# peterropac/Aegolius

Measured on AMD Instinct MI355X. Metric: Mpoints/sec SDF eval, 1024^3 grid, 10-prim smooth-union tree, higher is better.
Workload: dtype f32

## Files before the change

aegolius_amd/_engine.py:

```python
import atexit
import contextlib
import ctypes
import importlib.util
import os
import sys
import threading

import numpy as np

_HERE = os.path.dirname(os.path.abspath(__file__))
LIB_PATH = os.path.join(_HERE, "libsdfk.so")

MODE_AUTO, MODE_INTERPRET, MODE_SPECIALIZED, MODE_NOCULL = 0, 1, 2, 3
(FLAVOUR_PLAIN_ARRAY, FLAVOUR_PLAIN_GRID, FLAVOUR_TILE_ARRAY, FLAVOUR_TILE_GRID, FLAVOUR_TILE_MASK, FLAVOUR_ROWS_ARRAY,
 FLAVOUR_ROWS_GRID, FLAVOUR_ROWS_MASK, FLAVOUR_ROWS2D_ARRAY, FLAVOUR_ROWS2D_GRID, FLAVOUR_RAYS, FLAVOUR_OCCUPANCY) = range(12)
FLAVOUR_FLAGS = 0x100
FLAVOUR_XY = 0x200

_c = ctypes
_vp, _i64, _int, _sz = _c.c_void_p, _c.c_int64, _c.c_int, _c.c_size_t
_fp = _c.POINTER(_c.c_float)

SIGNATURES = {
    "sdfk_abi_version": (_int, []),
    "sdfk_device_count": (_int, []),
    "sdfk_last_error": (_c.c_char_p, []),
    "sdfk_program_create": (_vp, [_vp, _sz, _vp, _sz, _vp, _sz, _int]),
    "sdfk_program_destroy": (None, [_vp]),
    "sdfk_program_set_params": (_int, [_vp, _vp, _sz]),
    "sdfk_program_set_cull": (_int, [_vp, _vp, _sz, _vp]),
    "sdfk_program_source": (_c.c_char_p, [_vp]),
    "sdfk_program_compile_check": (_int, [_vp, _c.POINTER(_sz)]),
    "sdfk_program_chain_members": (_int, [_vp]),
    "sdfk_program_compile_flavour": (_int, [_vp, _int, _c.POINTER(_sz), _c.POINTER(_c.c_double)]),
    "sdfk_debug_compile_external": (_int, [_vp, _int, _c.POINTER(_sz)]),
    "sdfk_debug_jit_stats": (None, [_c.POINTER(_i64), _c.POINTER(_c.c_double)]),
    "sdfk_jit_drain": (None, []),
    "sdfk_jit_cancel": (None, []),
    "sdfk_debug_set_rtc_defs": (None, [_c.c_char_p]),
    "sdfk_eval_device": (_int, [_vp, _vp, _i64, _i64, _vp, _vp, _int]),
    "sdfk_eval_device_rows": (_int, [_vp, _vp, _i64, _i64, _i64, _vp, _vp, _int]),
    "sdfk_eval_device_rows2d": (_int, [_vp, _vp, _i64, _i64, _i64, _vp, _vp, _int]),
    "sdfk_eval_device_rows2d_xy": (_int, [_vp, _vp, _i64, _i64, _i64, _vp, _vp, _int]),
    "sdfk_debug_cells_stats": (None, [_int, _c.POINTER(_c.c_longlong)]),
    "sdfk_debug_rays_stats": (None, [_int, _c.POINTER(_c.c_longlong)]),
    "sdfk_eval_device_rows3d": (_int, [_vp, _vp, _i64, _i64, _i64, _i64, _i64, _vp, _vp, _int]),
    "sdfk_debug_row_masks": (_int, [_vp, _vp, _i64, _i64, _i64, _vp, _c.POINTER(_i64), _c.POINTER(_int), _vp]),
    "sdfk_eval_grid_sharded": (_int, [_vp, _vp, _i64, _vp, _i64, _vp, _i64, _int, _vp, _vp, _int]),
    "sdfk_eval_grid_sharded_device": (_int, [_vp, _vp, _i64, _vp, _i64, _vp, _i64, _int, _vp, _int, _vp, _int]),
    "sdfk_eval_device_aux": (_int, [_vp, _vp, _i64, _i64, _vp, _int, _i64, _vp, _vp, _int]),
    "sdfk_eval_grid_aux": (_int, [_vp, _vp, _i64, _vp, _i64, _vp, _i64, _i64, _i64, _vp, _int, _i64, _vp, _vp, _int]),
    "sdfk_field_min": (_int, [_vp, _i64, _c.POINTER(_c.c_float), _vp]),
    "sdfk_grid_box_average": (_int, [_vp, _i64, _i64, _i64, _int, _int, _int, _int, _vp, _vp]),
    "sdfk_grid_edge_detect": (_int, [_vp, _i64, _i64, _i64, _vp, _vp]),
    "sdfk_debug_box_variant": (_int, [_i64, _i64, _i64, _int, _int, _int, _c.POINTER(_int)]),
    "sdfk_grid_signed": (_int, [_vp, _i64, _i64, _i64, _c.c_float, _int, _vp, _vp]),
    "sdfk_grid_boundary_mask": (_int, [_vp, _i64, _c.c_float, _vp, _vp]),
    "sdfk_grid_signed_slab": (_int, [_vp, _i64, _i64, _vp, _i64, _i64, _i64, _int, _vp, _vp]),
    "sdfk_eval_host": (_int, [_vp, _vp, _int, _i64, _i64, _vp, _int, _int]),
    "sdfk_eval_host_resident": (_int, [_vp, _vp, _int, _i64, _i64, _vp, _int, _int]),
    "sdfk_field_select_scratch": (_sz, [_i64]),
    "sdfk_field_select": (_int, [_vp, _i64, _c.c_float, _vp, _i64, _c.POINTER(_i64), _vp, _vp]),
    "sdfk_field_select_finish": (_int, [_i64, _i64, _vp, _i64, _vp, _vp]),
    "sdfk_field_gradient": (_int, [_vp, _i64, _i64, _i64, _int, _int, _vp, _i64, _vp]),
    "sdfk_field_crossings_2d": (_int, [_vp, _vp, _i64, _i64, _i64, _c.c_double, _c.c_double, _c.c_double, _vp, _vp]),
    "sdfk_lcwg_eval": (_int, [_int, _vp, _vp, _i64, _i64, _i64, _c.c_double, _c.c_double, _int, _c.c_double, _vp, _vp, _i64,
                              _vp]),
    "sdfk_lcwg_old_eval": (_int, [_int, _vp, _i64, _vp, _i64, _c.c_double, _c.c_double, _vp, _i64, _vp]),
    "sdfk_eval_select_scratch": (_sz, [_i64, _i64]),
    "sdfk_eval_device_select": (_int, [_vp, _vp, _i64, _i64, _i64, _int, _c.c_float, _vp, _i64, _c.POINTER(_i64), _vp, _vp, _int]),
    "sdfk_eval_grid_select": (_int, [_vp, _vp, _i64, _vp, _i64, _vp, _i64, _i64, _i64, _c.c_float, _vp, _i64, _c.POINTER(_i64),
                                     _vp, _vp, _int]),
    "sdfk_eval_select_finish": (_int, [_vp, _i64, _i64, _int, _i64, _vp, _i64, _vp, _vp]),
    "sdfk_vec_eval_device": (_int, [_vp, _int, _vp, _i64, _i64, _vp, _int, _i64, _int, _vp, _i64, _vp]),
    "sdfk_vec_set_interpret": (None, [_int]),
    "sdfk_vec_source": (_c.c_char_p, [_vp, _int, _int, _int]),
    "sdfk_vec_compile_check": (_int, [_vp, _int, _int, _int, _c.POINTER(_sz)]),
    "sdfk_vec_eval_host": (_int, [_vp, _int, _vp, _int, _i64, _vp, _i64, _vp, _i64, _vp, _i64, _vp, _int, _int, _vp, _int]),
    "sdfk_eval_grid": (_int, [_vp, _vp, _i64, _vp, _i64, _vp, _i64, _i64, _i64, _vp, _vp, _int]),
    "sdfk_eval_grid_host": (_int, [_vp, _vp, _i64, _vp, _i64, _vp, _i64, _i64, _i64, _vp, _int, _int]),
    "sdfk_set_default_mode": (None, [_int]),
    "sdfk_debug_brick_masks": (_int, [_vp, _vp, _i64, _i64, _vp, _vp]),
    "sdfk_linspace_f32": (_int, [_c.c_double, _c.c_double, _i64, _vp]),
    "sdfk_point_tree_build": (_i64, [_vp, _i64, _int, _vp, _i64, _vp, _vp, _vp]),
    "sdfk_grid_fill": (_int, [_vp, _i64, _vp, _i64, _vp, _i64, _vp, _i64, _i64, _i64, _vp]),
    "sdfk_set_device": (_int, [_int]),
    "sdfk_malloc": (_vp, [_sz]),
    "sdfk_free": (_int, [_vp]),
    "sdfk_memcpy_h2d": (_int, [_vp, _vp, _sz]),
    "sdfk_memcpy_d2h": (_int, [_vp, _vp, _sz]),
    "sdfk_memcpy_d2d": (_int, [_vp, _vp, _sz]),
    "sdfk_sync": (_int, [_vp]),
    "sdfk_event_create": (_vp, []),
    "sdfk_event_destroy": (_int, [_vp]),
    "sdfk_event_record": (_int, [_vp, _vp]),
    "sdfk_event_elapsed_ms": (_int, [_vp, _vp, _fp]),
    "sdfk_stream_probe": (_int, [_vp, _i64, _i64, _vp, _vp]),
    "sdfk_dual_has_rule": (_int, [_int]),
    "sdfk_program_jvp_check": (_int, [_vp, _c.POINTER(_int)]),
    "sdfk_eval_jvp_device": (_int, [_vp, _vp, _i64, _i64, _vp, _int, _int, _vp, _vp, _i64, _vp]),
    "sdfk_value_jvp_device": (_int, [_int, _vp, _vp, _vp, _i64, _vp, _vp, _vp]),
    "sdfk_program_vjp_check": (_int, [_vp, _c.POINTER(_int), _c.POINTER(_i64)]),
    "sdfk_vjp_limits": (_int, [_c.POINTER(_int), _c.POINTER(_int)]),
    "sdfk_eval_vjp_device": (_int, [_vp, _vp, _i64, _i64, _vp, _int, _int, _vp, _vp, _vp, _vp]),
    "sdfk_points_bin": (_int, [_vp, _i64, _i64, _vp, _i64, _i64, _i64, _vp, _vp]),
    "sdfk_points_extent": (_int, [_vp, _i64, _i64, _i64, _vp, _vp]),
    "sdfk_points_fill": (_int, [_vp, _i64, _i64, _i64, _int, _i64, _i64, _i64, _vp]),
    "sdfk_points_widen": (_int, [_vp, _i64, _int, _vp, _vp]),
    "sdfk_field_isosurface_scratch": (_sz, [_i64, _i64, _i64]),
    "sdfk_field_isosurface": (_int, [_vp, _vp, _i64, _vp, _i64, _vp, _i64, _c.c_float, _c.POINTER(_i64), _c.POINTER(_i64), _vp,
                                     _vp]),
    "sdfk_field_isosurface_finish": (_int, [_vp, _i64, _i64, _i64, _c.c_float, _i64, _i64, _vp, _i64, _vp, _i64, _int, _vp,
                                            _vp]),
    "sdfk_field_contour2d_scratch": (_sz, [_i64, _i64]),
    "sdfk_field_contour2d": (_int, [_vp, _vp, _i64, _vp, _i64, _c.c_float, _c.POINTER(_i64), _c.POINTER(_i64), _vp, _vp]),
    "sdfk_field_contour2d_finish": (_int, [_vp, _i64, _i64, _c.c_float, _i64, _i64, _vp, _i64, _vp, _i64, _int, _vp, _vp]),
    "sdfk_eval_grid_isosurface_scratch": (_sz, [_i64, _i64, _i64]),
    "sdfk_eval_grid_isosurface": (_int, [_vp, _vp, _i64, _vp, _i64, _vp, _i64, _c.c_float, _c.POINTER(_i64), _c.POINTER(_i64),
                                         _vp, _vp, _int]),
    "sdfk_eval_grid_isosurface_finish": (_int, [_vp, _vp, _i64, _vp, _i64, _vp, _i64, _c.c_float, _i64, _i64, _vp, _i64, _vp,
                                                _i64, _int, _vp, _vp, _int]),
    "sdfk_eval_grid_contour2d_scratch": (_sz, [_i64, _i64]),
    "sdfk_eval_grid_contour2d": (_int, [_vp, _vp, _i64, _vp, _i64, _c.c_float, _c.POINTER(_i64), _c.POINTER(_i64), _vp, _vp,
                                        _int]),
    "sdfk_eval_grid_contour2d_finish": (_int, [_vp, _vp, _i64, _vp, _i64, _c.c_float, _i64, _i64, _vp, _i64, _vp, _i64, _int,
                                               _vp, _vp, _int]),
    "sdfk_program_rays_check": (_int, [_vp, _c.POINTER(_int)]),
    "sdfk_trace_rays_device": (_int, [_vp, _vp, _i64, _vp, _i64, _i64, _c.c_float, _c.c_float, _c.c_float, _c.c_float,
                                      _c.c_float, _int, _vp, _vp, _vp, _vp, _i64, _vp, _int]),
    "sdfk_trace_camera_device": (_int, [_vp, _vp, _int, _int, _int, _c.c_float, _c.c_float, _c.c_float, _c.c_float,
                                        _c.c_float, _int, _vp, _vp, _vp, _vp, _i64, _vp, _int]),
    "sdfk_eval_grid_occupancy_scratch": (_sz, [_i64, _i64, _i64, _i64]),
    "sdfk_eval_grid_occupancy": (_int, [_vp, _vp, _i64, _vp, _i64, _vp, _i64, _vp, _vp, _vp, _vp, _vp, _vp, _int, _c.c_float,
                                        _c.c_float, _vp, _vp, _i64, _c.POINTER(_i64), _c.POINTER(_i64), _fp, _vp, _int]),
    "sdfk_field_row_sums": (_int, [_vp, _i64, _i64, _vp, _vp, _vp]),
    "sdfk_field_redistance_scratch": (_sz, [_i64, _i64, _i64]),
    "sdfk_field_redistance": (_int, [_vp, _vp, _i64, _vp, _i64, _vp, _i64, _c.c_float, _c.c_float, _int, _vp, _vp,
                                     _c.POINTER(_i64), _fp, _vp]),
}


class SdfkError(RuntimeError):
    pass


_lib = None
_lock = threading.Lock()


def _share_torch_hip_runtime():
    if "torch" in sys.modules:
        return
    try:
        spec = importlib.util.find_spec("torch")
    except (ImportError, ValueError):
        spec = None
    if spec is None or not spec.submodule_search_locations:
        return
    libdir = os.path.join(list(spec.submodule_search_locations)[0], "lib")
    for name in ("libamdhip64.so", "libhiprtc.so"):
        path = os.path.join(libdir, name)
        if os.path.exists(path):
            try:
                ctypes.CDLL(path, mode=ctypes.RTLD_GLOBAL)
            except OSError:
# ... 617 lines not shown
```

aegolius_amd/csrc/sdfk.hip:

```cpp
#include <hip/hip_runtime.h>
#include <hip/hiprtc.h>

#include <chrono>
#include <algorithm>
#include <atomic>
#include <cmath>
#include <condition_variable>
#include <cstdio>
#include <cstdlib>
#include <cstring>
#include <deque>
#include <functional>
#include <map>
#include <memory>
#include <mutex>
#include <thread>
#include <string>
#include <vector>
#include <dirent.h>
#include <dlfcn.h>
#include <fcntl.h>
#include <signal.h>
#include <spawn.h>
#include <sys/wait.h>
// ... 474 lines not shown
        t.skip_b_ok = range_skippable(p, t.b0, t.b1, t.comb, c) ? 1 : 0;
        sites.push_back(t);
    }
    p->sites_all = sites;
    if (sites.size() > SDFK_MASK_SITES) {
        std::vector<size_t> order(sites.size());
        for (size_t i = 0; i < order.size(); ++i) order[i] = i;
        std::stable_sort(order.begin(), order.end(), [&](size_t x, size_t y) {
            return (sites[x].a1 - sites[x].a0) + (sites[x].b1 - sites[x].b0) > (sites[y].a1 - sites[y].a0) + (sites[y].b1 - sites[y].b0);
        });
        order.resize(SDFK_MASK_SITES);
        std::sort(order.begin(), order.end());
        std::vector<sdfk_cullsite> widest;
        for (size_t i : order) widest.push_back(sites[i]);
        sites.swap(widest);
    }
    p->sites = sites;
    p->chain_members = sdfk_chain_mode(g_ops, SDFK_OP_COUNT, p->code.data(), p->code.size() / 2, p->result_reg, p->sites_all);
    p->chain_mode = p->chain_members > 0;
    p->key.append("|cull");
    for (const sdfk_cullsite& t : p->sites_all) {
        p->key.append(reinterpret_cast<const char*>(&t), sizeof t);
    }
    return 0;
}

extern "C" const char* sdfk_program_source(sdfk_program* p) {
    if (!p) return nullptr;
    std::lock_guard<std::mutex> lk(p->mu);
    if (p->source.empty())
        p->source = sdfk_generate_source(g_ops, SDFK_OP_COUNT, p->code.data(), p->code.size() / 2, p->result_reg,
                                         p->sites, SDFK_FL_ALL, &p->sites_all);
    return p->source.c_str();
}

static std::atomic<int> g_twaves_override{0}, g_rwbricks_override{0};
static int tile_waves() {
    static int v = [] { const char* e = getenv("SDFK_TWAVES"); int t = e ? atoi(e) : 4; return (t >= 1 && t <= 16) ? t : 4; }();
    const int o = g_twaves_override.load();
    return o ? o : v;
}
static int tile_wbricks() {
    static int v = [] {
        const char* e = getenv("SDFK_WBRICKS");
        int t = e ? atoi(e) : 4;
        if (t < 1 || t > 32) t = 4;
        return t;
    }();
    return v;
}
static int tile_points() { return tile_waves() * tile_wbricks() * 128; }
static std::atomic<int> g_rwaves_override{0};
static int rows_waves(const sdfk_program*) {
    if (const int o = g_rwaves_override.load()) return o;
    return 4;
}
static int rows_wbricks(const sdfk_program* p);
static long long big_program_limit() {
    static const long long v = [] {
        const char* e = getenv("SDFK_BIG_PROGRAM");
        const long long t = e ? atoll(e) : 300;
        return t > 0 ? t : 300;
    }();
    return v;
}
static int rows_geo(const sdfk_program* p) {
    const bool big = p && !p->chain_mode && (long long)(p->code.size() / 2) > big_program_limit();
    return rows_wbricks(p) | (rows_waves(p) << 4) | (big ? 1 << 16 : 0);
}
static int rows_wbricks(const sdfk_program* p) {
    static int forced = [] { const char* e = getenv("SDFK_RWBRICKS"); int t = e ? atoi(e) : 0; return (t >= 1 && t <= 16) ? t : 0; }();
    if (const int o = g_rwbricks_override.load()) return o;
    if (forced) return forced;
    if (p && p->chain_mode) return p->chain_members <= 64 ? 2 : 1;
    return 2;
}
struct RowGeom {
    unsigned L, nchunk, nbricks;
    long long R;
    long long row0;
    int yrows;
    unsigned prow, seg0, nb0, bpp;
    unsigned inv_nchunk, inv_bpp;
};
static bool rows_geometry(long long n, long long row_len, RowGeom* g, long long plane_rows = 0, long long plane_phase = 0,
                          bool planes_on = false) {
    if (row_len < 32 || row_len > 0x7fffffffLL || n <= 0 || n % row_len != 0) return false;
    const long long R = n / row_len, brows = 16;
    const long long nchunk = (row_len % 32 == 0) ? row_len / 32 : (row_len + 62) / 32;
    long long prow = plane_rows, seg0 = 0;
    static const bool plane_blocks = [] { const char* e = getenv("SDFK_PLANE_BLOCKS"); return e && e[0] == '1'; }();
    if (!(plane_blocks || planes_on) || prow <= 0 || prow >= R || prow > 0x7fffffffLL) {
        prow = R > 0x7fffffffLL ? 0 : R;
        if (prow == 0) return false;
    } else if (plane_phase > 0) {
        seg0 = std::min(R, (prow - plane_phase % prow) % prow);
    }
    const long long nb0 = (seg0 + brows - 1) / brows, bpp = (prow + brows - 1) / brows;
    const long long planes = (R - seg0 + prow - 1) / prow;
    const long long nb = nchunk * (nb0 + planes * bpp);
    if (nb > 0x7fffffffLL - 1024) return false;
    g->L = (unsigned)row_len;
    g->nchunk = (unsigned)nchunk;
    g->nbricks = (unsigned)nb;
    g->R = R;
    g->row0 = 0;
    g->yrows = 0;
    g->prow = (unsigned)prow;
    g->seg0 = (unsigned)seg0;
    g->nb0 = (unsigned)nb0;
    g->bpp = (unsigned)bpp;
    g->inv_nchunk = (unsigned)std::min<unsigned long long>(0xffffffffull, (1ull << 32) / (unsigned long long)nchunk);
    g->inv_bpp = (unsigned)std::min<unsigned long long>(0xffffffffull, (1ull << 32) / (unsigned long long)bpp);
    return true;
}
static int tile_threads() { return 64 * tile_waves(); }
static std::string rtc_cache_dir() {
    static const std::string dir = [] {
        std::string d;
        if (const char* e = getenv("SDFK_CACHE_DIR")) {
            d = e;
            if (d.empty() || d == "off" || d == "0") return std::string();
        } else if (const char* x = getenv("XDG_CACHE_HOME"); x && *x) {
            d = std::string(x) + "/sdfk";
        } else if (const char* h = getenv("HOME"); h && *h) {
            (void)mkdir((std::string(h) + "/.cache").c_str(), 0700);
            d = std::string(h) + "/.cache/sdfk";
        } else {
            return std::string();
        }
        (void)mkdir(d.c_str(), 0700);
        return d;
    }();
    return dir;
}
static std::string rtc_cache_path(const std::string& src, const std::string& opts) {
    const std::string dir = rtc_cache_dir();
    if (dir.empty()) return std::string();
    int major = 0, minor = 0;
    (void)hiprtcVersion(&major, &minor);
    unsigned long long h = 1469598103934665603ull;
    auto mix = [&](const std::string& t) {
        for (unsigned char c : t) {
            h ^= c;
            h *= 1099511628211ull;
        }
    };
    mix(src);
    mix(opts);
    mix(std::to_string(major) + "." + std::to_string(minor) + "/abi" + std::to_string(SDFK_ABI_VERSION));
    char name[96];
    snprintf(name, sizeof name, "/sdfk-%016llx-%zu.co", h, src.size());
    return dir + name;
}
static const unsigned long long kCacheMagic = 0x53444643'4f424a31ull;
static unsigned long long fnv1a(const char* p, size_t n) {
    unsigned long long h = 1469598103934665603ull;
    for (size_t i = 0; i < n; ++i) {
        h ^= (unsigned char)p[i];
        h *= 1099511628211ull;
    }
    return h;
}
static bool rtc_cache_read(const std::string& path, std::vector<char>* out) {
    if (path.empty()) return false;
    FILE* f = fopen(path.c_str(), "rb");
    if (!f) return false;
    bool ok = false;
    if (fseek(f, 0, SEEK_END) == 0) {
        const long size = ftell(f);
        if (size > 24 && fseek(f, 0, SEEK_SET) == 0) {
            out->resize((size_t)size);
            ok = fread(out->data(), 1, (size_t)size, f) == (size_t)size;
            if (ok) {
                unsigned long long tr[3];
                memcpy(tr, out->data() + size - 24, 24);
                ok = tr[0] == kCacheMagic && tr[1] == (unsigned long long)(size - 24) && tr[2] == fnv1a(out->data(), (size_t)size - 24);
                out->resize((size_t)size - 24);
            }
        }
    }
    fclose(f);
    if (!ok) {
        out->clear();
        (void)remove(path.c_str());
    } else {
        (void)utimes(path.c_str(), nullptr);
    }
    return ok;
}
static void rtc_cache_evict(const std::string& dir) {
    static const long long cap = [] {
        const char* e = getenv("SDFK_CACHE_MAX_MB");
        const long long v = e ? atoll(e) : 512;
        return (v > 0 ? v : 512) * (1ll << 20);
    }();
// ... 760 lines not shown
    DevState* d = nullptr;
    int rc = ensure_resident(p, device, stream, &d);
    if (rc) return rc;

    long long n4 = vec_ok ? (n / 4) * 4 : 0;
    long long tail = n - n4;

    static const long long spec_limit = [] {
        const char* e = getenv("SDFK_SPECIALIZE_LIMIT");
        const long long v = e ? atoll(e) : 1200;
        return v > 0 ? v : 1200;
    }();
    static const long long rows_limit = [] {
        const char* e = getenv("SDFK_ROWS_LIMIT");
        const long long v = e ? atoll(e) : 1200;
        return v > 0 ? v : 1200;
    }();
    if (mode == SDFK_MODE_AUTO && (long long)(p->code.size() / 2) > spec_limit && p->interp_ok && !p->chain_mode && !d_flags)
        mode = SDFK_MODE_INTERPRET;

    RowGeom rg;
    int flavour = arr ? SDFK_FL_PLAIN_ARRAY : SDFK_FL_PLAIN_GRID;
    const long long grow = grid ? (grid->n2 > 1 ? (long long)grid->n2 : (long long)grid->n1) : 0;
    if (!p->sites.empty() && mode != SDFK_MODE_NOCULL && mode != SDFK_MODE_INTERPRET) {
        if (arr && rows_geometry(n, row_len, &rg, (flat || d_flags) ? 0 : plane_rows, plane_phase, p->chain_mode))
            flavour = (flat || xy) ? SDFK_FL_ROWS2D_ARRAY : SDFK_FL_ROWS_ARRAY;
        else if (arr && vec_ok && !p->chain_mode && !d_flags && !xy) flavour = SDFK_FL_TILE_ARRAY;
        else if (grid && grid->start % grow == 0 &&
                 rows_geometry(n, grow, &rg, (grid->n2 > 1 && !d_flags) ? (long long)grid->n1 : 0,
                               grid->n2 > 1 ? (grid->start / grow) % (long long)grid->n1 : 0, p->chain_mode))
            flavour = grid->n2 > 1 ? SDFK_FL_ROWS_GRID : SDFK_FL_ROWS2D_GRID;
        else if (grid && vec_ok && !p->chain_mode && !d_flags) flavour = SDFK_FL_TILE_GRID;
        if (!p->chain_mode && (long long)(p->code.size() / 2) > rows_limit &&
            (flavour == SDFK_FL_ROWS_ARRAY || flavour == SDFK_FL_ROWS2D_ARRAY || flavour == SDFK_FL_ROWS_GRID || flavour == SDFK_FL_ROWS2D_GRID)) {
            const bool is_arr = arr != nullptr;
            if (vec_ok && !d_flags && !xy) flavour = is_arr ? SDFK_FL_TILE_ARRAY : SDFK_FL_TILE_GRID;
            else if (!d_flags) flavour = is_arr ? SDFK_FL_PLAIN_ARRAY : SDFK_FL_PLAIN_GRID;
        }
    }
    std::shared_ptr<SpecModule> sk;
    if (mode != SDFK_MODE_INTERPRET) {
        static const bool async_jit = [] { const char* e = getenv("SDFK_ASYNC_JIT"); return !(e && e[0] == '0'); }();
        const bool wait = mode != SDFK_MODE_AUTO || !p->interp_ok || !async_jit;
        std::string err;
        sk = get_module(p, device, flavour, wait, &err, (d_flags ? 1 : 0) | (xy ? 2 : 0));
        if (sk && sk->failed) {
            if (mode == SDFK_MODE_SPECIALIZED || !p->interp_ok)
                return fail(-3, "specialised kernel unavailable: " + err);
            static bool warned = false;
            if (!warned) {
                fprintf(stderr, "[sdfk] hiprtc specialisation failed, using the interpreter kernel: %s\n", err.c_str());
                warned = true;
            }
            sk.reset();
        }
    }
    if (!sk && !p->interp_ok)
        return fail(-4, "program needs more registers than the interpreter kernel has (use the specialised mode)");

    const float* prm = d->d_params;
    const float* tab = d->d_tables;
    if (sk) {
        if (flavour == SDFK_FL_ROWS_ARRAY || flavour == SDFK_FL_ROWS_GRID || flavour == SDFK_FL_ROWS2D_ARRAY ||
            flavour == SDFK_FL_ROWS2D_GRID) {
            const unsigned per_tile = (unsigned)(rows_waves(p) * rows_wbricks(p));
            const unsigned tiles = ((rg.nbricks + per_tile - 1) / per_tile + 127u) & ~127u;
            const unsigned rthreads = 64u * (unsigned)rows_waves(p);
            CellsArg cells{};
            const bool with_cells = p->chain_mode && sk->fn[1] != nullptr;
            if (arr) {
                const float* co = arr->co;
                long long stride = arr->stride;
                if (with_cells) {
                    void* src[] = {&co, &stride};
                    rc = prepare_cells(p, d, sk->fn[1], rg, src, 2, prm, tab, stream, &cells);
                    if (rc) return rc;
                }
                void* args[] = {&prm, &tab, &co, &stride, &rg, &d_out, &d_flags, &thr_key, &cells};
                HIPCHK(hipModuleLaunchKernel(sk->fn[0], tiles, 1, 1, rthreads, 1, 1, 0, stream, args, nullptr));
            } else {
                SrcGrid g = *grid;
                rg.row0 = grid->start / grow;
                rg.yrows = grid->n2 > 1 ? 0 : 1;
                if (with_cells) {
                    void* src[] = {&g};
                    rc = prepare_cells(p, d, sk->fn[1], rg, src, 1, prm, tab, stream, &cells);
                    if (rc) return rc;
                }
                void* args[] = {&prm, &tab, &g, &rg, &d_out, &d_flags, &thr_key, &cells};
                HIPCHK(hipModuleLaunchKernel(sk->fn[0], tiles, 1, 1, rthreads, 1, 1, 0, stream, args, nullptr));
            }
            return 0;
        }
        if (flavour == SDFK_FL_TILE_ARRAY || flavour == SDFK_FL_TILE_GRID) {
            const unsigned tiles = (unsigned)((n + tile_points() - 1) / tile_points());
            if (arr) {
                const float* co = arr->co;
                long long stride = arr->stride;
                void* args[] = {&prm, &tab, &co, &stride, &n, &d_out};
                HIPCHK(hipModuleLaunchKernel(sk->fn[0], tiles, 1, 1, tile_threads(), 1, 1, 0, stream, args, nullptr));
            } else {
                SrcGrid g = *grid;
                void* args[] = {&prm, &tab, &g, &n, &d_out};
                HIPCHK(hipModuleLaunchKernel(sk->fn[0], tiles, 1, 1, tile_threads(), 1, 1, 0, stream, args, nullptr));
            }
            return 0;
        }
        if (arr) {
            const float* co = arr->co;
            long long stride = arr->stride;
            if (n4) {
                long long off = 0;
                void* args[] = {&prm, &tab, &co, &stride, &off, &n4, &d_out, &aux, &aux_stride, &d_flags, &thr_key};
                HIPCHK(hipModuleLaunchKernel(sk->fn[0], blocks_for(n4, 4), 1, 1, SDFK_BLOCK, 1, 1, 0, stream, args,
                                             nullptr));
            }
            if (tail) {
                long long off = n4;
                void* args[] = {&prm, &tab, &co, &stride, &off, &tail, &d_out, &aux, &aux_stride, &d_flags, &thr_key};
                HIPCHK(hipModuleLaunchKernel(sk->fn[1], blocks_for(tail, 1), 1, 1, SDFK_BLOCK, 1, 1, 0, stream, args,
                                             nullptr));
            }
        } else {
            SrcGrid g = *grid;
            if (n4) {
                long long off = 0;
                void* args[] = {&prm, &tab, &g, &off, &n4, &d_out, &aux, &aux_stride, &d_flags, &thr_key};
                HIPCHK(hipModuleLaunchKernel(sk->fn[0], blocks_for(n4, 4), 1, 1, SDFK_BLOCK, 1, 1, 0, stream, args,
                                             nullptr));
            }
            if (tail) {
                long long off = n4;
                void* args[] = {&prm, &tab, &g, &off, &tail, &d_out, &aux, &aux_stride, &d_flags, &thr_key};
                HIPCHK(hipModuleLaunchKernel(sk->fn[1], blocks_for(tail, 1), 1, 1, SDFK_BLOCK, 1, 1, 0, stream, args,
                                             nullptr));
            }
        }
        return 0;
    }
    if (d_flags) return fail(-3, "fused selection needs the specialised kernels");
    const int n_instr = (int)(p->code.size() / 2);
    const long long zero = 0;
    auto launch = [&](auto src, int vec, long long off, long long cnt) {
        using SRC = decltype(src);
        const dim3 grid(blocks_for(cnt, vec)), block(SDFK_BLOCK);
#define SDFK_INTERP_GO(VEC, NC, NV) hipLaunchKernelGGL((sdfk_interp_kernel<VEC, NC, NV, SRC>), grid, block, 0, stream, d->d_code, \
                                                        n_instr, prm, tab, src, off, cnt, d_out, p->result_reg, aux, aux_stride)
        if (vec == 4) {
            if (p->interp_small) SDFK_INTERP_GO(4, SDFK_NC_SMALL, SDFK_NV_SMALL);
            else SDFK_INTERP_GO(4, SDFK_NC, SDFK_NV);
        } else {
            if (p->interp_small) SDFK_INTERP_GO(1, SDFK_NC_SMALL, SDFK_NV_SMALL);
            else SDFK_INTERP_GO(1, SDFK_NC, SDFK_NV);
        }
#undef SDFK_INTERP_GO
    };
    if (arr) {
        if (n4) launch(*arr, 4, zero, n4);
        if (tail) launch(*arr, 1, n4, tail);
    } else {
        if (n4) launch(*grid, 4, zero, n4);
        if (tail) launch(*grid, 1, n4, tail);
    }
    HIPCHK(hipGetLastError());
    return 0;
}
// ... 82 lines not shown
    DevState* d = nullptr;
    int rc = ensure_resident(p, device, stream, &d);
    if (rc) return rc;
    std::string err;
    std::shared_ptr<SpecModule> sk = get_module(p, device, SDFK_FL_ROWS_MASK, true, &err);
    if (!sk || sk->failed) return fail(-3, "specialised kernel unavailable: " + err);
    const float* prm = d->d_params;
    const float* tab = d->d_tables;
    long long stride = row_stride;
    void* args[] = {&prm, &tab, &d_co, &stride, &rg, &d_masks};
    const unsigned per_tile = (unsigned)(rows_waves(p) * rows_wbricks(p));
    HIPCHK(hipModuleLaunchKernel(sk->fn[0], (rg.nbricks + per_tile - 1) / per_tile, 1, 1, 64 * rows_waves(p), 1, 1, 0, stream,
                                 args, nullptr));
    return 0;
}

extern "C" int sdfk_debug_brick_masks(sdfk_program* p, const float* d_co, int64_t n, int64_t row_stride,
                                      uint64_t* d_masks, void* stream_) {
    if (!p || !d_co || !d_masks) return fail(-1, "sdfk_debug_brick_masks: null argument");
    if (!(aligned16(d_co) && row_stride % 4 == 0 && row_stride >= n && n > 0))
        return fail(-1, "sdfk_debug_brick_masks: needs 16-byte aligned rows");
    if (p->sites.empty()) return fail(-2, "sdfk_debug_brick_masks: program has no cull sites");
    if (p->chain_mode) return fail(-2, "sdfk_debug_brick_masks: chain-mode programs have no line-brick flavour");
    hipStream_t stream = (hipStream_t)stream_;
    int device = 0;
    HIPCHK(hipGetDevice(&device));
    DevState* d = nullptr;
    int rc = ensure_resident(p, device, stream, &d);
    if (rc) return rc;
    std::string err;
    std::shared_ptr<SpecModule> sk = get_module(p, device, SDFK_FL_TILE_MASK, true, &err);
    if (!sk || sk->failed) return fail(-3, "specialised kernel unavailable: " + err);
    const float* prm = d->d_params;
    const float* tab = d->d_tables;
    long long stride = row_stride, nn = n;
    void* args[] = {&prm, &tab, &d_co, &stride, &nn, &d_masks};
    HIPCHK(hipModuleLaunchKernel(sk->fn[0], (unsigned)((n + tile_points() - 1) / tile_points()), 1, 1, tile_threads(),
                                 1, 1, 0, stream, args, nullptr));
    return 0;
}

extern "C" int sdfk_linspace_f32(double lo, double hi, int64_t n, float* out) {
    if (n < 0 || (n > 0 && !out)) return fail(-1, "sdfk_linspace_f32: bad arguments");
    if (n == 0) return 0;
    if (n == 1) {
        out[0] = (float)lo;
        return 0;
    }
    const double div = (double)(n - 1);
    const double delta = hi - lo;
    const double step = delta / div;
    for (int64_t i = 0; i < n; ++i) {
        volatile double t = (step != 0.0) ? (double)i * step : ((double)i / div) * delta;
        out[i] = (float)(t + lo);
    }
    out[n - 1] = (float)hi;
    return 0;
}

struct AxisTables {
    float* d = nullptr;
    ~AxisTables() {
        if (d) (void)hipFree(d);
    }
};

static int upload_axes(const float* ax0, int64_t n0, const float* ax1, int64_t n1, const float* ax2, int64_t n2,
                       hipStream_t stream, AxisTables* t, SrcGrid* g, int64_t start) {
    if (!ax0 || !ax1 || !ax2 || n0 < 1 || n1 < 1 || n2 < 1) return fail(-1, "grid axes missing or empty");
    if (n1 > 0x7fffffff || n2 > 0x7fffffff) return fail(-1, "grid axis too long");
    HIPCHK(hipMalloc(&t->d, (size_t)(n0 + n1 + n2) * sizeof(float)));
    HIPCHK(hipMemcpyAsync(t->d, ax0, (size_t)n0 * sizeof(float), hipMemcpyHostToDevice, stream));
    HIPCHK(hipMemcpyAsync(t->d + n0, ax1, (size_t)n1 * sizeof(float), hipMemcpyHostToDevice, stream));
    HIPCHK(hipMemcpyAsync(t->d + n0 + n1, ax2, (size_t)n2 * sizeof(float), hipMemcpyHostToDevice, stream));
    g->ax0 = t->d;
    g->ax1 = t->d + n0;
    g->ax2 = t->d + n0 + n1;
    g->n1 = (unsigned)n1;
    g->n2 = (unsigned)n2;
    g->start = start;
    return 0;
}

extern "C" int sdfk_eval_grid(sdfk_program* p, const float* ax0, int64_t n0, const float* ax1, int64_t n1,
                              const float* ax2, int64_t n2, int64_t start, int64_t count, float* d_out, void* stream,
                              int mode) {
    if (!d_out) return fail(-1, "sdfk_eval_grid: null output");
    if (start < 0 || count < 0 || start + count > n0 * n1 * n2) return fail(-1, "sdfk_eval_grid: range outside the grid");
    AxisTables t;
    SrcGrid g;
    int rc = upload_axes(ax0, n0, ax1, n1, ax2, n2, (hipStream_t)stream, &t, &g, start);
    if (rc) return rc;
    rc = run(p, nullptr, &g, count, d_out, stream, mode, aligned16(d_out));
    if (rc) return rc;
    HIPCHK(hipStreamSynchronize((hipStream_t)stream));
    return 0;
}

extern "C" int sdfk_eval_grid_aux(sdfk_program* p, const float* ax0, int64_t n0, const float* ax1, int64_t n1,
                                  const float* ax2, int64_t n2, int64_t start, int64_t count, const float* d_aux, int n_aux,
                                  int64_t aux_stride, float* d_out, void* stream, int mode) {
    if (!p || !d_out) return fail(-1, "sdfk_eval_grid_aux: null pointer");
    if (start < 0 || count < 0 || start + count > n0 * n1 * n2) return fail(-1, "sdfk_eval_grid_aux: range outside the grid");
    if (n_aux < p->n_aux) return fail(-1, "sdfk_eval_grid_aux: the program reads more auxiliary fields than were passed");
    AxisTables t;
    SrcGrid g;
    int rc = upload_axes(ax0, n0, ax1, n1, ax2, n2, (hipStream_t)stream, &t, &g, start);
    if (rc) return rc;
    rc = run(p, nullptr, &g, count, d_out, stream, mode, aligned16(d_out), 0, d_aux, aux_stride);
    if (rc) return rc;
    HIPCHK(hipStreamSynchronize((hipStream_t)stream));
    return 0;
}

extern "C" int sdfk_eval_grid_host(sdfk_program* p, const float* ax0, int64_t n0, const float* ax1, int64_t n1,
                                   const float* ax2, int64_t n2, int64_t start, int64_t count, float* out, int device,
                                   int mode) {
    if (!p) return fail(-1, "null program");
    if (count < 0 || (count > 0 && !out)) return fail(-1, "sdfk_eval_grid_host: bad arguments");
    if (start < 0 || start + count > n0 * n1 * n2) return fail(-1, "sdfk_eval_grid_host: range outside the grid");
    if (count == 0) return 0;
    HIPCHK(hipSetDevice(device));
    int64_t chunk = std::min<int64_t>(count, (int64_t)1 << 27);
    const int64_t grow = n2 > 1 ? n2 : n1;
    if (start % grow == 0 && chunk > grow) chunk = chunk / grow * grow;
    float* d_out = nullptr;
    HIPCHK(hipMalloc(&d_out, (size_t)chunk * sizeof(float)));
    AxisTables t;
    SrcGrid g;
    int rc = upload_axes(ax0, n0, ax1, n1, ax2, n2, nullptr, &t, &g, start);
    for (int64_t s = 0; s < count && rc == 0; s += chunk) {
        const int64_t m = std::min(chunk, count - s);
        g.start = start + s;
        rc = run(p, nullptr, &g, m, d_out, nullptr, mode, true);
        if (rc == 0 && hipMemcpy(out + s, d_out, (size_t)m * sizeof(float), hipMemcpyDeviceToHost) != hipSuccess)
            rc = fail(-6, "sdfk_eval_grid_host: device-to-host copy failed");
    }
    (void)hipFree(d_out);
    return rc;
}

extern "C" int sdfk_eval_grid_sharded(sdfk_program* p, const float* ax0, int64_t n0, const float* ax1, int64_t n1,
                                      const float* ax2, int64_t n2, int n_shards, const int* devices, float* out,
                                      int mode) {
    if (!p || !out) return fail(-1, "sdfk_eval_grid_sharded: null argument");
    if (n_shards < 1 || n_shards > 64) return fail(-1, "sdfk_eval_grid_sharded: 1..64 shards");
    if (!ax0 || !ax1 || !ax2 || n0 < 1 || n1 < 1 || n2 < 1) return fail(-1, "grid axes missing or empty");
    int n_dev = 0;
    if (hipGetDeviceCount(&n_dev) != hipSuccess || n_dev < 1) return fail(-8, "sdfk_eval_grid_sharded: no HIP device");
    const int64_t total = n0 * n1 * n2, unit = n2 > 1 ? n2 : n1;
    const int64_t per = (total / unit / n_shards) * unit;
    std::vector<int> rc((size_t)n_shards, 0);
    std::vector<std::string> msg((size_t)n_shards);
    std::vector<std::thread> workers;
    for (int d = 0; d < n_shards; ++d) {
        const int dev = devices ? devices[d] : d % n_dev;
        if (dev < 0 || dev >= n_dev) return fail(-1, "sdfk_eval_grid_sharded: device index out of range");
    }
    for (int d = 0; d < n_shards; ++d) {
        const int dev = devices ? devices[d] : d % n_dev;
        const int64_t start = d * per, count = d < n_shards - 1 ? per : total - start;
        workers.emplace_back([=, &rc, &msg] {
            rc[(size_t)d] = count > 0 ? sdfk_eval_grid_host(p, ax0, n0, ax1, n1, ax2, n2, start, count, out + start, dev, mode) : 0;
            if (rc[(size_t)d]) msg[(size_t)d] = sdfk_last_error();
        });
    }
    for (std::thread& t : workers) t.join();
    for (int d = 0; d < n_shards; ++d)
        if (rc[(size_t)d]) return fail(rc[(size_t)d], "shard " + std::to_string(d) + ": " + msg[(size_t)d]);
    return 0;
}

extern "C" int sdfk_eval_grid_sharded_device(sdfk_program* p, const float* ax0, int64_t n0, const float* ax1, int64_t n1,
                                             const float* ax2, int64_t n2, int n_shards, const int* devices,
                                             int gather_device, float* d_full, int mode) {
    if (!p || !d_full) return fail(-1, "sdfk_eval_grid_sharded_device: null argument");
    if (n_shards < 1 || n_shards > 64) return fail(-1, "sdfk_eval_grid_sharded_device: 1..64 shards");
    if (!ax0 || !ax1 || !ax2 || n0 < 1 || n1 < 1 || n2 < 1) return fail(-1, "grid axes missing or empty");
    int n_dev = 0;
    if (hipGetDeviceCount(&n_dev) != hipSuccess || n_dev < 1) return fail(-8, "sdfk_eval_grid_sharded_device: no HIP device");
    if (gather_device < 0 || gather_device >= n_dev) return fail(-1, "sdfk_eval_grid_sharded_device: gather device out of range");
    for (int d = 0; d < n_shards; ++d) {
        const int dev = devices ? devices[d] : d % n_dev;
        if (dev < 0 || dev >= n_dev) return fail(-1, "sdfk_eval_grid_sharded_device: device index out of range");
    }
    const int64_t total = n0 * n1 * n2, unit = n2 > 1 ? n2 : n1;
    const int64_t per = (total / unit / n_shards) * unit;
    std::vector<int> rc((size_t)n_shards, 0);
    std::vector<std::string> msg((size_t)n_shards);
    std::vector<std::thread> workers;
    for (int d = 0; d < n_shards; ++d) {
        const int dev = devices ? devices[d] : d % n_dev;
        const int64_t start = d * per, count = d < n_shards - 1 ? per : total - start;
        workers.emplace_back([=, &rc, &msg] {
            auto shard = [&]() -> int {
                if (count <= 0) return 0;
                HIPCHK(hipSetDevice(dev));
                hipStream_t stream = nullptr;
                HIPCHK(hipStreamCreateWithFlags(&stream, hipStreamNonBlocking));
                static const bool force_copy = [] { const char* e = getenv("SDFK_FORCE_PEER_COPY"); return e && e[0] == '1'; }();
                const bool in_place = dev == gather_device && !force_copy;
                float* d_slab = in_place ? d_full + start : nullptr;
                int r = 0;
                if (!d_slab && hipMalloc(&d_slab, (size_t)count * sizeof(float)) != hipSuccess) r = fail(-5, "out of device memory for the slab");
                if (r == 0) r = sdfk_eval_grid(p, ax0, n0, ax1, n1, ax2, n2, start, count, d_slab, stream, mode);
                if (r == 0 && !in_place) {
                    if (hipMemcpyPeerAsync(d_full + start, gather_device, d_slab, dev, (size_t)count * sizeof(float), stream) != hipSuccess ||
                        hipStreamSynchronize(stream) != hipSuccess)
                        r = fail(-6, "peer copy of the slab failed");
                }
                if (!in_place && d_slab) (void)hipFree(d_slab);
                (void)hipStreamDestroy(stream);
                return r;
            };
            rc[(size_t)d] = shard();
            if (rc[(size_t)d]) msg[(size_t)d] = sdfk_last_error();
        });
    }
    for (std::thread& t : workers) t.join();
    for (int d = 0; d < n_shards; ++d)
        if (rc[(size_t)d]) return fail(rc[(size_t)d], "shard " + std::to_string(d) + ": " + msg[(size_t)d]);
    return 0;
}

extern "C" int sdfk_grid_fill(float* d_co, int64_t row_stride, const float* ax0, int64_t n0, const float* ax1,
                              int64_t n1, const float* ax2, int64_t n2, int64_t start, int64_t count, void* stream) {
    if (!d_co) return fail(-1, "sdfk_grid_fill: null output");
    if (row_stride < count) return fail(-1, "sdfk_grid_fill: row stride smaller than count");
    if (start < 0 || count < 0 || start + count > n0 * n1 * n2) return fail(-1, "sdfk_grid_fill: range outside the grid");
    if (count == 0) return 0;
    AxisTables t;
    SrcGrid g;
    int rc = upload_axes(ax0, n0, ax1, n1, ax2, n2, (hipStream_t)stream, &t, &g, start);
    if (rc) return rc;
    hipLaunchKernelGGL(sdfk_gridfill_kernel, dim3(blocks_for(count, 4)), dim3(SDFK_BLOCK), 0, (hipStream_t)stream, g,
                       (long long)count, d_co, (long long)row_stride);
    HIPCHK(hipGetLastError());
    HIPCHK(hipStreamSynchronize((hipStream_t)stream));
    return 0;
}

template <typename T>
static int64_t detect_row_len(const T* co, int64_t n, int64_t stride, bool* flat, int64_t* plane_rows) {
    const int64_t scan = std::min<int64_t>(n, (int64_t)1 << 22);
    const T *x = co, *y = co + stride, *z = co + 2 * stride;
    int64_t a = 0, b = 0;
    *flat = false;
    *plane_rows = 0;
    for (int64_t i = 1; i < scan && (!a || !b); ++i) {
        if (!b && x[i] != x[0]) b = i;
        if (!a && (x[i] != x[0] || y[i] != y[0])) a = i;
    }
    if (a >= 32 && n % a == 0) {
        if (b > a && b % a == 0) *plane_rows = b / a;
        return a;
    }
    if (b >= 32 && n % b == 0) {
        *flat = z[0] == (T)0 && z[b - 1] == (T)0 && z[n - 1] == (T)0;
        return b;
    }
    return 0;
}

struct HostSlot {
    float *h_co = nullptr, *h_out = nullptr, *d_co = nullptr, *d_out = nullptr;
    hipStream_t stream = nullptr;
    hipEvent_t done = nullptr;
    int64_t pending_start = -1, pending_count = 0;
};
struct HostStage {
    std::mutex mu;
    int64_t chunk = 0;
    HostSlot slot[2];
};
static std::mutex g_stage_mu;
static std::map<int, std::unique_ptr<HostStage>> g_stage;
static int host_threads() {
    static int v = [] {
        const char* e = getenv("SDFK_HOST_THREADS");
        int t = e ? atoi(e) : 0;
        if (t < 1) t = std::min(8, std::max(1, (int)std::thread::hardware_concurrency() / 4));
        return std::min(t, 64);
    }();
    return v;
}
template <typename F>
static void parallel_ranges(int64_t count, F fn) {
    const int t = (int)std::min<int64_t>(host_threads(), std::max<int64_t>(1, count >> 18));
// ... 229 lines not shown
```

aegolius_amd/csrc/sdfk_access.h:

```cpp
#ifndef SDFK_ACCESS_H
#define SDFK_ACCESS_H

#define SDFK_BLOCK 256

struct SrcArray {
    const float* __restrict__ co;
    long long stride;
};
struct SrcGrid {
    const float* __restrict__ ax0;
    const float* __restrict__ ax1;
    const float* __restrict__ ax2;
    unsigned n1, n2;
    long long start;
};

typedef float sdfk_f4 __attribute__((ext_vector_type(4)));
static __device__ __forceinline__ float4 sdfk_stream_load4(const float* p) {
    const sdfk_f4 v = __builtin_nontemporal_load(reinterpret_cast<const sdfk_f4*>(p));
    return make_float4(v.x, v.y, v.z, v.w);
}
static __device__ __forceinline__ void sdfk_stream_store4(float* p, float a, float b, float c, float d) {
    const sdfk_f4 v = {a, b, c, d};
    __builtin_nontemporal_store(v, reinterpret_cast<sdfk_f4*>(p));
}

template <int VEC>
static __device__ __forceinline__ void sdfk_load(const SrcArray& s, long long block_base, unsigned lane_off,
                                                 V3 (&p)[VEC]) {
    const long long i = block_base + lane_off;
    if constexpr (VEC == 4) {
        const float4 x = sdfk_stream_load4(s.co + i);
        const float4 y = sdfk_stream_load4(s.co + s.stride + i);
#ifdef SDFK_XY
        const float4 z = make_float4(0.0f, 0.0f, 0.0f, 0.0f);
#else
        const float4 z = sdfk_stream_load4(s.co + 2 * s.stride + i);
#endif
        p[0] = {x.x, y.x, z.x};
        p[1] = {x.y, y.y, z.y};
        p[2] = {x.z, y.z, z.z};
        p[3] = {x.w, y.w, z.w};
    } else {
#pragma unroll
#ifdef SDFK_XY
        for (int v = 0; v < VEC; ++v) p[v] = {s.co[i + v], s.co[s.stride + i + v], 0.0f};
#else
        for (int v = 0; v < VEC; ++v) p[v] = {s.co[i + v], s.co[s.stride + i + v], s.co[2 * s.stride + i + v]};
#endif
    }
}

template <int VEC>
static __device__ __forceinline__ void sdfk_load(const SrcGrid& s, long long block_base, unsigned lane_off,
                                                 V3 (&p)[VEC]) {
    const unsigned long long base = (unsigned long long)(s.start + block_base);
    const unsigned long long row = base / s.n2;
    const unsigned iz0 = (unsigned)(base - row * s.n2);
    const unsigned long long ix0 = row / s.n1;
    const unsigned iy0 = (unsigned)(row - ix0 * s.n1);
#pragma unroll
    for (int v = 0; v < VEC; ++v) {
        const unsigned t = iz0 + lane_off + v;
        const unsigned cz = t / s.n2;
        const unsigned iz = t - cz * s.n2;
        const unsigned ty = iy0 + cz;
        const unsigned cy = ty / s.n1;
        const unsigned iy = ty - cy * s.n1;
        p[v] = {s.ax0[ix0 + cy], s.ax1[iy], s.ax2[iz]};
    }
}

static __host__ __device__ __forceinline__ unsigned sdfk_sel_key(float v) {
    unsigned u = __builtin_bit_cast(unsigned, v);
    if ((u & 0x7fffffffu) > 0x7f800000u) return 0xffffffffu;
    if (u == 0x80000000u) u = 0u;
    return (u & 0x80000000u) ? ~u : (u | 0x80000000u);
}
template <int VEC>
static __device__ __forceinline__ void sdfk_store_flags(unsigned* __restrict__ flags, long long i, unsigned nib, bool active) {
    if constexpr (VEC == 4) {
        const unsigned lane = __builtin_amdgcn_workitem_id_x() & 63u;
        unsigned w = nib << (4u * (lane & 7u));
        w |= __shfl_xor(w, 1);
        w |= __shfl_xor(w, 2);
        w |= __shfl_xor(w, 4);
        if ((lane & 7u) == 0u && active) flags[i >> 5] = w;
    } else {
        if (active && nib) atomicOr(&flags[i >> 5], nib << (unsigned)(i & 31));
    }
}

template <int VEC>
static __device__ __forceinline__ void sdfk_store(float* __restrict__ out, long long i, const float (&v)[VEC]) {
    if constexpr (VEC == 4) {
        sdfk_stream_store4(out + i, v[0], v[1], v[2], v[3]);
    } else {
#pragma unroll
// ... 6 lines not shown
```

aegolius_amd/csrc/sdfk_codegen.cpp:

```cpp
#include "sdfk_codegen.h"

#include <algorithm>
#include <cstdio>
#include <cstring>
#include <map>
#include <set>

#include "sdfk_embedded.inc"

std::string sdfk_vector_prelude() { return std::string(kEmbeddedDevice) + "\n" + kEmbeddedVecdev + "\n"; }

static const char kWrappers[] = R"SDFKW(
template <int VEC, typename SRC>
static __device__ __forceinline__ void sdfk_body(const float* __restrict__ PRM, const float* __restrict__ TAB,
                                                 const SRC& src, long long off, long long n,
                                                 float* __restrict__ out, const float* __restrict__ aux,
                                                 long long aux_stride, unsigned* __restrict__ flags, unsigned thr) {
    const long long block_base = (long long)sdfk_bx() * (SDFK_BLOCK * VEC);
    const unsigned lane_off = sdfk_tx() * VEC;
#ifdef SDFK_FLAGS                                              // the flag-writing build of this flavour (its own code object:
    {                                                          // carried as a run-time branch it cost the field kernels registers)
        const bool active = block_base + lane_off < n;
        unsigned nib = 0u;
        if (active) {
// ... 555 lines not shown
// One tile per workgroup; many short-lived workgroups per CU sit in different phases at any time, which is
// what overlaps the memory phase (A) with the VALU phases (B, C). Two persistent variants (register prefetch
// per CU the phases run in lockstep and the single-wave probe leaves the CU idle.
template <typename SRC>
static __device__ __forceinline__ void sdfk_tile_kernel(const float* __restrict__ PRM, const float* __restrict__ TAB,
                                                        const SRC& src, long long n, float* __restrict__ out) {
    __shared__ __attribute__((aligned(16))) sdfk_tilemeta meta;
    sdfk_tile_prepare(PRM, TAB, src, n, &meta);
    sdfk_tile_evaluate(PRM, TAB, src, n, (long long)sdfk_bx() * SDFK_TILE, &meta, out, sdfk_tx() & 63,
                       sdfk_tx() >> 6);
}
)SDFKT";
static const char kTileArray[] = R"SDFKT(
extern "C" __global__ __launch_bounds__(SDFK_TTHREADS) void sdfk_spec_t(
    const float* __restrict__ PRM, const float* __restrict__ TAB, const float* __restrict__ co, long long stride,
    long long n, float* __restrict__ out) {
    const SrcArray s = {co, stride};
    sdfk_tile_kernel(PRM, TAB, s, n, out);
}
)SDFKT";
static const char kTileGrid[] = R"SDFKT(
// the same on a regular grid expanded from three per-axis tables: no coordinate array at all (4 B/point)
extern "C" __global__ __launch_bounds__(SDFK_TTHREADS) void sdfk_spec_tg(
    const float* __restrict__ PRM, const float* __restrict__ TAB, SrcGrid g, long long n, float* __restrict__ out) {
    sdfk_tile_kernel(PRM, TAB, g, n, out);
}
)SDFKT";
static const char kTileMask[] = R"SDFKT(
// debugging / test aid: the skip masks of every brick (2 bits per site: bit 2k = skip first operand,
// bit 2k+1 = skip second operand; bit 63 = x/y-constant run, bit 62 = two such runs)
extern "C" __global__ __launch_bounds__(SDFK_TTHREADS) void sdfk_spec_tmask(
    const float* __restrict__ PRM, const float* __restrict__ TAB, const float* __restrict__ co, long long stride,
    long long n, unsigned long long* __restrict__ masks) {
    __shared__ __attribute__((aligned(16))) sdfk_tilemeta meta;
    const SrcArray s = {co, stride};
    sdfk_tile_prepare(PRM, TAB, s, n, &meta);
    for (int b = sdfk_tx(); b < SDFK_NBRICK; b += SDFK_TTHREADS)
        masks[(long long)sdfk_bx() * SDFK_NBRICK + b] = sdfk_brick_mask(&meta, b);
}
)SDFKT";


static const char kSimtGeometry[] = R"SDFKR(
#ifndef SDFK_RWBRICKS
#define SDFK_RWBRICKS 2
#endif
#ifndef SDFK_RWAVES
#define SDFK_RWAVES 4
#endif
#ifndef SDFK_NSUB                        // sub-bricks (probe centres) per brick: 16 = 4 rows x 8 points, 8 = 8 rows x 8, 4 = 16 rows x 8
// becomes the cost: 4 centres up to 96 leaves (round 4, smooth unions of n primitives at 513^3, 1 -> 4 centres: n = 40
#define SDFK_NSUB ((SDFK_NLEAF <= 32 && 8 * SDFK_RWBRICKS <= 64) ? 8 : ((SDFK_NLEAF <= 96 && 4 * SDFK_RWBRICKS <= 64) ? 4 : 1))
#endif
#define SDFK_NCEN (SDFK_RWAVES * SDFK_RWBRICKS * SDFK_NSUB)
static_assert(SDFK_NSUB == 1 || SDFK_NSUB == 4 || SDFK_NSUB == 8 || SDFK_NSUB == 16, "1, 4, 8 or 16 probe centres per brick");
static_assert(SDFK_NCEN <= 64 * SDFK_RWAVES, "one fold lane per probe centre");
)SDFKR";

static const char kRowsKernel[] = R"SDFKR(
#ifndef SDFK_RWBRICKS
#define SDFK_RWBRICKS 2
#endif
#ifndef SDFK_RWAVES
#define SDFK_RWAVES 4                           // waves per workgroup (host launch code must agree: sdfk.hip)
#endif
#define SDFK_RZ 32
#define SDFK_RLPR (SDFK_RZ / (2 * SDFK_NP))     // lanes per row in phase C
#define SDFK_RROWS (64 / SDFK_RLPR)             // rows per brick
#define SDFK_RBRICK (SDFK_RZ * SDFK_RROWS)
#define SDFK_RLOADS (SDFK_RROWS / 8)            // load instructions per array and brick
#define SDFK_RNBRICK (SDFK_RWAVES * SDFK_RWBRICKS)
#ifndef SDFK_CHUNK
#define SDFK_CHUNK 16                            // chain mode: children whose parameters are staged in LDS at a time
#endif
#ifndef SDFK_STAGE_MIN
#define SDFK_STAGE_MIN 2                         // ... when more than this many survive on the brick
#endif
#ifndef SDFK_CHAIN_STAGED                        // Round 3 staged the survivors' parameters in LDS for chains of more than 64
#define SDFK_CHAIN_STAGED 0                      // children (three dependent loads per child: kind, base, parameters). With the
#endif                                           // survivors kept as RECORDS (round 4) one load is left between the list and the
                                                 // 4096: 2.21 -> 2.11 (SDFK_STAGE_MIN=64 against 2); -DSDFK_CHAIN_STAGED=1 brings it back
static_assert(SDFK_NP == 2 || SDFK_NP == 4, "2 or 4 packed pairs per lane");
static_assert(SDFK_RNBRICK <= 64 * SDFK_RWAVES, "one probe lane per brick");

typedef float sdfk_f4u __attribute__((ext_vector_type(4), aligned(4)));

#ifdef SDFK_CELLS
#ifndef SDFK_ALIST_CAP
#define SDFK_ALIST_CAP (SDFK_NLEAF < 192 ? SDFK_NLEAF : 192)     // survivors a brick's list holds in LDS
#endif
#define SDFK_ALL_ALIVE 0xffffffffu
#define SDFK_LIST_ALIVE 0xfffffffeu
#endif
struct sdfk_rowmeta {
    float z[SDFK_RNBRICK][SDFK_RBRICK];         // [row of the brick][point of the window]
    float2 xy[SDFK_RNBRICK][SDFK_RROWS];
    float4 bound[SDFK_RNBRICK];
    unsigned long long mask[SDFK_NMASK][SDFK_RNBRICK];   // two bits per site: SDFK_NMASK x 32 sites (2 words up to 64 sites)
    unsigned uniform[SDFK_RNBRICK];
#if defined(SDFK_SIMT) && !defined(SDFK_CELLS)
    float4 cen[SDFK_NCEN];                      // probe centres (x, y, z, radius): SDFK_NSUB per brick
    float leafval[SDFK_NLEAF * SDFK_NCEN];      // [leaf][centre]: every leaf of the tree at every centre
#endif
#ifdef SDFK_CHAIN
#ifdef SDFK_CELLS
    unsigned alist[SDFK_RNBRICK][SDFK_ALIST_CAP];                      // RECORDS of the children that run, in order
    uint2 aspan[SDFK_RNBRICK];                                         // more survivors than that: the cell's whole list runs (nalive = LIST)
    unsigned inside[SDFK_RNBRICK];                                     // every point of the brick lies in its cell's sphere
#else
    unsigned short alist[SDFK_RNBRICK][SDFK_NLEAF];                    // the children that run, in order
#endif
    unsigned nalive[SDFK_RNBRICK];
#if SDFK_CHAIN_STAGED
    float cprm[SDFK_RNBRICK][SDFK_CHUNK][SDFK_NPLMAX];                  // parameters of the chunk of children being evaluated
    unsigned cgrp[SDFK_RNBRICK][SDFK_CHUNK];                            // ... and their kinds
#endif
#endif
#ifdef SDFK_LDSPAD
    float pad[SDFK_LDSPAD / 4];                 // experiment: a larger LDS footprint per workgroup
#endif
};
struct sdfk_rowgeom {
    unsigned L, nchunk, nbricks;                // row length, windows per row, bricks in total
    long long R;                                // rows
    long long row0;                             // grid flavour: global row index of the first row of the slab
    int yrows;                                  // grid flavour, 2-D grid (n2 == 1): rows run along the second axis
    unsigned prow, seg0, nb0, bpp;              // planes of prow rows after a first partial plane of seg0 rows (nb0 blocks);
                                                // bpp blocks per plane: a block never holds rows of two planes
    unsigned inv_nchunk, inv_bpp;               // floor(2^32 / nchunk), floor(2^32 / bpp): divisions as one v_mul_hi
};
#ifdef SDFK_CELLS
// Candidate lists (chain mode). The bricks are grouped into CELLS in index space — 2^lx plane slots x 2^ly row blocks x
// 2^lz windows — and a pre-pass (sdfk_spec_cells) leaves per cell a bounding sphere, derived from the coordinates of the
// cell's eight corner points, and the LIST of members that can be the minimum somewhere in that sphere (the global-minimum
// rule of sdfk_chain_fold at the cell's radius; cells of a coarser level first, so that a fine cell only looks at its
// parent's list). A brick then probes the members on its cell's list instead of all of them — after checking, point by
// point, that it really lies inside the sphere: the corner points bound the cell only if the array is the lattice its
// layout hints say it is, and a brick that fails the check (or whose cell ran out of list space) probes every member,
// as before. Whatever the input, a member that is dropped cannot be the minimum at any point of the brick.
struct sdfk_celllevel {
    unsigned lx, ly, lz;                        // log2 of the cell size in plane slots, row blocks, windows
    unsigned ncx, ncy, ncz;                     // cells along each of them
    unsigned xoff;                              // slot number of the first whole plane (2^lx when a partial plane leads, else 0)
    unsigned pad;
};
struct sdfk_cells {
    sdfk_celllevel lv;                          // the level the bricks look at (the finest)
    const float4* __restrict__ sph;             // per cell: centre, radius (< 0: no such cell)
    const uint2* __restrict__ span;             // per cell: first entry, entries (SDFK_ALL_ALIVE: no list — probe every member)
    const unsigned* __restrict__ cand;          // the lists: one RECORD per member (sdfk_member_record: kind and parameter block)
    unsigned enabled, ncells;
};
#endif
// a / d for wave-uniform a, with inv = floor(2^32 / d) from the host: the estimate is never too large and at most a few
// units too small (a * (2^32 - inv * d) < 2^32 * d for every brick count the host accepts), the loop repairs it.
// (A plain 32-bit division is ~35 vector instructions; this kernel has two per brick.)
static __device__ __forceinline__ unsigned sdfk_udiv(unsigned a, unsigned d, unsigned inv) {
    unsigned q = __umulhi(a, inv);
    while (a - q * d >= d) ++q;
    return __builtin_amdgcn_readfirstlane(q);
}
// rows [r0, rend) of row block rb (wave-uniform): 16 consecutive rows of ONE plane, fewer at the end of a plane
// (slot, blk: plane slot — 0 = the leading partial plane, whole planes from 0 as well; the caller adds its offset — and the
//  block's index within it)
static __device__ __forceinline__ void sdfk_block_rows(const sdfk_rowgeom& g, unsigned rb, long long& r0, long long& rend,
                                                       unsigned* slot = nullptr, unsigned* blk = nullptr) {
    // ONE plane (no plane hint, flat grids, plane blocks not asked for): blocks of 16 consecutive rows, nothing to divide
    if (g.nb0 == 0u && (long long)g.prow >= g.R) {
        r0 = (long long)rb * SDFK_RROWS;
        rend = g.R;
        if (slot) { *slot = 0u; *blk = rb; }
        return;
    }
    if (rb < g.nb0) {
        r0 = (long long)rb * SDFK_RROWS;
        rend = g.seg0;
        if (slot) { *slot = 0xffffffffu; *blk = rb; }
    } else {
        const unsigned k = rb - g.nb0;
        const unsigned pl = sdfk_udiv(k, g.bpp, g.inv_bpp);
        const long long base = (long long)g.seg0 + (long long)pl * g.prow;
        r0 = base + (long long)(k - pl * g.bpp) * SDFK_RROWS;
        rend = base + g.prow < g.R ? base + g.prow : g.R;
        if (slot) { *slot = pl; *blk = k - pl * g.bpp; }
    }
}

// Rows are cut into WINDOWS of 32 points that are aligned in the flat array (128-byte lines when the array is):
// window k of a row starts at flat index 32 * (floor(row * L / 32) + k), i.e. up to 31 points before the row
// (tools/rowstream.hip), whole lines cost nothing. Elements outside the row are replaced by the nearest point
// of the row (duplicates keep bounds and the uniformity test valid) and never stored; that only happens in the
// first and the last windows of a row ("edge" chunks, wave-uniform).
static __device__ __forceinline__ bool sdfk_interior(unsigned L, unsigned k) {      // wave-uniform
    return (L & 31u) == 0u || (k >= 1u && 32u * k + 32u <= L);
}
static __device__ __forceinline__ float4 sdfk_win_quad(const float* __restrict__ rowp, int z, int last, bool interior) {
    if (interior) {
        const sdfk_f4u v = __builtin_nontemporal_load(reinterpret_cast<const sdfk_f4u*>(rowp + z));
        return make_float4(v.x, v.y, v.z, v.w);
    }
    // edge window, branch-free on purpose: per-lane branches around the loads (whole quad / one value / mixed)
    return make_float4(rowp[min(max(z, 0), last)], rowp[min(max(z + 1, 0), last)], rowp[min(max(z + 2, 0), last)],
                       rowp[min(max(z + 3, 0), last)]);
}
// the 4 points [z, z+4) of row `row` (row = r0 + dr, r0 wave-uniform) as three quads
static __device__ __forceinline__ void sdfk_rows_fetch(const SrcArray& s, const sdfk_rowgeom& g, long long r0, int dr, int z,
                                                       bool interior, float4& X, float4& Y, float4& Z) {
    const float* p = s.co + (r0 + dr) * (long long)g.L;
    const int last = (int)g.L - 1;
    X = sdfk_win_quad(p, z, last, interior);
    Y = sdfk_win_quad(p + s.stride, z, last, interior);
#ifdef SDFK_XY                                                    // two-row coordinates (z = 0 by contract): 12 B/point
    Z = make_float4(0.0f, 0.0f, 0.0f, 0.0f);
#else
    Z = sdfk_win_quad(p + 2 * s.stride, z, last, interior);
#endif
}
// regular grid: row -> (ix, iy) with one wave-uniform division per brick; z from the third axis table
static __device__ __forceinline__ void sdfk_rows_fetch(const SrcGrid& s, const sdfk_rowgeom& g, long long r0, int dr, int z,
                                                       bool interior, float4& X, float4& Y, float4& Z) {
    const unsigned long long g0 = (unsigned long long)(g.row0 + r0);
    if (g.yrows) {                                                 // (x, y, z) = (ax0[row], ax1[point], ax2[0])
        const float x = s.ax0[g0 + (unsigned)dr], zc = s.ax2[0];
        X = make_float4(x, x, x, x);
        Y = sdfk_win_quad(s.ax1, z, (int)g.L - 1, interior);
        Z = make_float4(zc, zc, zc, zc);
        return;
    }
    unsigned long long ix = g0 / s.n1;
    unsigned iy = (unsigned)(g0 - ix * s.n1) + (unsigned)dr;
    while (iy >= s.n1) { iy -= s.n1; ++ix; }
    const float x = s.ax0[ix], y = s.ax1[iy];
    X = make_float4(x, x, x, x);
    Y = make_float4(y, y, y, y);
    Z = sdfk_win_quad(s.ax2, z, (int)g.L - 1, interior);
}
static __device__ __forceinline__ float sdfk_prev_lane(float v) {   // value of lane-1 within a row of 16 lanes
    return __builtin_bit_cast(float, __builtin_amdgcn_update_dpp(__builtin_bit_cast(int, v), __builtin_bit_cast(int, v), 0x111, 0xf, 0xf, false));
}
// point index (in its row) of the first point of window k of local row `row`, plus e0
static __device__ __forceinline__ int sdfk_win_z(long long row, unsigned L, unsigned k, int e0, long long* flat) {
    const long long rl = row * (long long)L;
    const long long f = (((rl >> 5) + k) << 5) + e0;
    *flat = f;
    return (int)(f - rl);
}

// phase A, part 1: issue the loads of one brick (wave-uniform r0, k); 8 rows x 32 points per instruction
struct sdfk_rowregs {
    float4 X[SDFK_RLOADS], Y[SDFK_RLOADS], Z[SDFK_RLOADS];
};
template <typename SRC>
static __device__ __forceinline__ void sdfk_rows_load(const SRC& s, const sdfk_rowgeom& g, long long r0, long long rend,
                                                      unsigned k, int lane, sdfk_rowregs& r) {
    // SDFK_FLAT (flat grids: rows run along y, z = 0 everywhere): the roles of y and z are swapped from here to the
    // end of phase A — r.Y holds z (the coordinate a row shares, which must be exactly 0) and r.Z holds y (the one
    // that varies along the row) — so that "uniform", the staging and the bounding sphere work unchanged
    const bool interior = sdfk_interior(g.L, k);
#pragma unroll
    for (int t = 0; t < SDFK_RLOADS; ++t) {
        int dr = 8 * t + (lane >> 3);
        if (r0 + dr >= rend) dr = (int)(rend - 1 - r0);
        long long flat;
        const int z = sdfk_win_z(r0 + dr, g.L, k, 4 * (lane & 7), &flat);
        #ifdef SDFK_FLAT
        sdfk_rows_fetch(s, g, r0, dr, z, interior, r.X[t], r.Z[t], r.Y[t]);
#else
        sdfk_rows_fetch(s, g, r0, dr, z, interior, r.X[t], r.Y[t], r.Z[t]);
#endif
    }
}
// phase A, part 2: z and the row heads to LDS, "every row has one x and one y", bounding sphere
// (SDFK_CELLS: S = sphere of the brick's cell, with y and z swapped for SDFK_FLAT like the registers; the brick also learns
//  whether every one of its points lies inside it)
#ifdef SDFK_CELLS
#define SDFK_CELL_ARG , float4 S
#else
#define SDFK_CELL_ARG
#endif
static __device__ __forceinline__ void sdfk_rows_bounds(const sdfk_rowregs& r, int lane, sdfk_rowmeta* meta, int b SDFK_CELL_ARG) {
#ifdef SDFK_ABLATE_BOUNDS
    *reinterpret_cast<float4*>(&meta->z[b][(lane >> 3) * SDFK_RZ + 4 * (lane & 7)]) = r.Z[0];
    if (SDFK_RLOADS > 1) *reinterpret_cast<float4*>(&meta->z[b][(8 + (lane >> 3)) * SDFK_RZ + 4 * (lane & 7)]) = r.Z[SDFK_RLOADS - 1];
    if ((lane & 7) == 0) { meta->xy[b][lane >> 3] = make_float2(r.X[0].x, r.Y[0].x); meta->xy[b][SDFK_RROWS - 8 + (lane >> 3)] = make_float2(r.X[SDFK_RLOADS - 1].x, r.Y[SDFK_RLOADS - 1].x); }
    if (lane == 0) { meta->bound[b] = make_float4(0.f, 0.f, 0.f, 1.f); meta->uniform[b] = 1u; }
#ifdef SDFK_CELLS
    if (lane == 0) meta->inside[b] = S.w > 0.0f ? 1u : 0u;
#endif
    return;
#endif
    bool uni = true;
#pragma unroll
    for (int t = 0; t < SDFK_RLOADS; ++t) {
        *reinterpret_cast<float4*>(&meta->z[b][(8 * t + (lane >> 3)) * SDFK_RZ + 4 * (lane & 7)]) = r.Z[t];
        const float px = sdfk_prev_lane(r.X[t].x), py = sdfk_prev_lane(r.Y[t].x);
        const bool head = (lane & 7) == 0;
        uni = uni && r.X[t].x == r.X[t].y && r.X[t].x == r.X[t].z && r.X[t].x == r.X[t].w && r.Y[t].x == r.Y[t].y &&
              r.Y[t].x == r.Y[t].z && r.Y[t].x == r.Y[t].w && (head || (px == r.X[t].x && py == r.Y[t].x));
#ifdef SDFK_FLAT
        uni = uni && r.Y[t].x == 0.0f;                             // (M2 * 0 drops out of every root transform exactly)
#endif
        if (head) meta->xy[b][8 * t + (lane >> 3)] = make_float2(r.X[t].x, r.Y[t].x);
    }
    const bool uniform = __ballot(uni) == ~0ull;
#if defined(SDFK_SIMT) && SDFK_NSUB > 1
    // bricks of whole row segments are bounded per SUB-brick by the probe lanes (sdfk_sub_centre, from the staged
    // coordinates): the sphere around the whole brick is only needed for the others
    if (uniform) {
        if (lane == 0) {
            meta->uniform[b] = 1u;
#pragma unroll
            for (int w = 0; w < SDFK_NMASK; ++w) meta->mask[w][b] = ~0ull;
        }
        return;
    }
#endif
    const float cx = 0.5f * (sdfk_lane(r.X[0].x, 0) + sdfk_lane(r.X[SDFK_RLOADS - 1].w, 63));
    const float cy = 0.5f * (sdfk_lane(r.Y[0].x, 0) + sdfk_lane(r.Y[SDFK_RLOADS - 1].w, 63));
    const float cz = 0.5f * (sdfk_lane(r.Z[0].x, 0) + sdfk_lane(r.Z[SDFK_RLOADS - 1].w, 63));
    float d2 = 0.0f;
#ifdef SDFK_CELLS
    float d2s = 0.0f;                                // the same maximum about the CELL's centre
#endif
    if (uniform) {                                   // one x, y per row segment: |p - c|^2 = dxy^2 + max |z - cz|^2
#pragma unroll
        for (int t = 0; t < SDFK_RLOADS; ++t) {
            const float dx = r.X[t].x - cx, dy = r.Y[t].x - cy;
            const float zm = sd_rawmax(sd_rawmax(sd_abs(r.Z[t].x - cz), sd_abs(r.Z[t].y - cz)),
                                       sd_rawmax(sd_abs(r.Z[t].z - cz), sd_abs(r.Z[t].w - cz)));
            d2 = sd_rawmax(d2, sd_fma(zm, zm, sd_fma(dx, dx, dy * dy)));
// ... 7 lines not shown
    } else {
#pragma unroll
        for (int t = 0; t < SDFK_RLOADS; ++t) {
            const f2 xa = {r.X[t].x, r.X[t].y}, xb = {r.X[t].z, r.X[t].w}, ya = {r.Y[t].x, r.Y[t].y}, yb = {r.Y[t].z, r.Y[t].w};
            const f2 za = {r.Z[t].x, r.Z[t].y}, zb = {r.Z[t].z, r.Z[t].w};
            const f2 ax = xa - cx, ay = ya - cy, az = za - cz, bx = xb - cx, by = yb - cy, bz = zb - cz;
            const f2 da = sd_fma(ax, ax, sd_fma(ay, ay, az * az)), db = sd_fma(bx, bx, sd_fma(by, by, bz * bz));
            d2 = sd_rawmax(d2, sd_rawmax(sd_rawmax(da.x, da.y), sd_rawmax(db.x, db.y)));
#ifdef SDFK_CELLS
            const f2 ex = xa - S.x, ey = ya - S.y, ez = za - S.z, fx = xb - S.x, fy = yb - S.y, fz = zb - S.z;
            const f2 ea = sd_fma(ex, ex, sd_fma(ey, ey, ez * ez)), eb = sd_fma(fx, fx, sd_fma(fy, fy, fz * fz));
            d2s = sd_rawmax(d2s, sd_rawmax(sd_rawmax(ea.x, ea.y), sd_rawmax(eb.x, eb.y)));
#endif
        }
    }
    const float r2 = sdfk_wave_max(d2);
#ifdef SDFK_CELLS
    // inside: max |p - S| <= radius of S, with room for the rounding of the distances (relative 1e-5; S.w < 0: no cell)
    const float rs2 = sdfk_wave_max(d2s);
    if (lane == 0) meta->inside[b] = (S.w > 0.0f && 1.00002f * sqrtf(rs2) <= S.w) ? 1u : 0u;
#endif
    if (lane == 0) {
#ifdef SDFK_FLAT
        meta->bound[b] = make_float4(cx, cz, cy, 1.00001f * sqrtf(r2) + 1e-30f);
#else
        meta->bound[b] = make_float4(cx, cy, cz, 1.00001f * sqrtf(r2) + 1e-30f);
#endif
        meta->uniform[b] = uniform ? 1u : 0u;
#ifdef SDFK_SIMT
#pragma unroll
        for (int w = 0; w < SDFK_NMASK; ++w) meta->mask[w][b] = ~0ull;   // the fold lanes AND their decisions into these
#endif
    }
}
#if defined(SDFK_SIMT) && SDFK_NSUB > 1
// Probe centre `sb` of brick b whose rows each have one x and one y: the sub-brick is rows [r0, r0 + RPS) x points
// [i0, i0 + ZPS) of the window; sphere around the midpoint of its first and last point, radius = the exact maximum
// over its points (read back from the staged coordinates), so any input is bounded correctly — on a regular grid
// 4 rows x 8 points have a quarter of the brick's radius.
static __device__ __forceinline__ float4 sdfk_sub_centre(const sdfk_rowmeta* meta, unsigned b, unsigned sb) {
    constexpr int NZP = 4, NRP = SDFK_NSUB / NZP, RPS = SDFK_RROWS / NRP, ZPS = SDFK_RZ / NZP;
    static_assert(ZPS % 4 == 0 && RPS >= 1, "sub-brick shape");
    int r0 = (int)(sb / NZP) * RPS, r1 = r0 + RPS;
    const int i0 = (int)(sb % NZP) * ZPS;
    if constexpr (NRP == 2) {
        // A brick whose 16 rows come from TWO planes of the grid (1 row block in 32 at 513^3: the last rows of one plane,
        // y near its maximum, and the first rows of the next, y near its minimum) is split where x changes instead of in the
        // middle: each part lies in one plane and is bounded tightly; split in the middle, the part that holds the plane
        // change spans the whole y extent and nothing of the brick could be culled.
        const float x0 = meta->xy[b][0].x;
        if (__builtin_bit_cast(unsigned, x0) != __builtin_bit_cast(unsigned, meta->xy[b][SDFK_RROWS - 1].x)) {
            int s = 1;
            while (s < SDFK_RROWS - 1 && __builtin_bit_cast(unsigned, meta->xy[b][s].x) == __builtin_bit_cast(unsigned, x0)) ++s;
            r0 = sb / NZP ? s : 0;
            r1 = sb / NZP ? SDFK_RROWS : s;
        }
    }
    const float2 pa = meta->xy[b][r0], pe = meta->xy[b][r1 - 1];
    const float za = meta->z[b][r0 * SDFK_RZ + i0], ze = meta->z[b][(r1 - 1) * SDFK_RZ + i0 + ZPS - 1];
    const float cx = 0.5f * (pa.x + pe.x), cy = 0.5f * (pa.y + pe.y), cz = 0.5f * (za + ze);
    float r2 = 0.0f;
#pragma unroll 1
    for (int rr = r0; rr < r1; ++rr) {
        const int r = rr - r0;
        const float2 p = meta->xy[b][r0 + r];
        const float dx = p.x - cx, dy = p.y - cy;
        float zm = 0.0f;
#pragma unroll
        for (int i = 0; i < ZPS; i += 4) {
            const float4 q = *reinterpret_cast<const float4*>(&meta->z[b][(r0 + r) * SDFK_RZ + i0 + i]);
            zm = sd_rawmax(sd_rawmax(zm, sd_abs(q.x - cz)), sd_rawmax(sd_abs(q.y - cz), sd_rawmax(sd_abs(q.z - cz), sd_abs(q.w - cz))));
        }
        r2 = sd_rawmax(r2, sd_fma(zm, zm, sd_fma(dx, dx, dy * dy)));
    }
    const float rho = 1.00001f * sqrtf(r2) + 1e-30f;
#ifdef SDFK_FLAT
    return make_float4(cx, cz, cy, rho);                         // (the staged coordinate is y, xy holds (x, z = 0))
#else
    return make_float4(cx, cy, cz, rho);
#endif
}
#endif

#if defined(SDFK_CHAIN) && !defined(SDFK_CELLS)
// Chain mode, one WAVE per brick: which children run on this brick, from the leaf values at its centre. A hard min (max:
// signs flipped, e_k = +-d_k) is exact, associative and commutative, so the ORDER of the chain does not matter for a
// decision: child k can be dropped wherever some other child j stays below it on the whole brick, and with j = the child
// that is smallest at the centre that is guaranteed by e_k - m >= thr, m = min_j e_j, thr = K rho + margins with
// K = the largest Lipschitz sum of the chain (any pair). No prefix minimum, no "restart" level: one reduction for m, then
// 64 children per step — compare, ballot, and the survivors written as a LIST in index order, so that the evaluation
// never looks at a child it skips and still combines the others in the chain's order. (Tighter than the sequential rule,
// which compares a child with its predecessors only.)
static __device__ __forceinline__ void sdfk_chain_fold(sdfk_rowmeta* meta, int b, int lane) {
    const float4 cc = meta->bound[b];
    const float rho = cc.w, cmag = 1e-6f * (fabsf(cc.x) + fabsf(cc.y) + fabsf(cc.z) + rho);
    constexpr int NW = (SDFK_NLEAF + 63) / 64;
    float m = 3.0e38f;
#pragma unroll 4
    for (int j = 0; j < NW; ++j) {
        const int k = 64 * j + lane;
        if (k < SDFK_NLEAF) m = fminf(m, SDFK_CHAIN_SGN * meta->leafval[k * SDFK_NCEN + b]);
    }
#pragma unroll
    for (int o = 1; o < 64; o <<= 1) m = fminf(m, __shfl_xor(m, o));
    const float thr0 = 1.0001f * SDFK_CHAIN_KMAX * rho + SDFK_CHAIN_KMAX * cmag + 1e-6f * (1.0f + fabsf(m));
    int n_out = 0;
#pragma unroll 1
    for (int j = 0; j < NW; ++j) {
        const int k = 64 * j + lane;
        const bool in = k < SDFK_NLEAF;
        const float e = in ? SDFK_CHAIN_SGN * meta->leafval[k * SDFK_NCEN + b] : 3.0e38f;
        const bool run = in && !(e - m >= thr0 + 1e-6f * fabsf(e));
        const unsigned long long bits = __ballot(run);
        if (run) meta->alist[b][n_out + __builtin_popcountll(bits & ((1ull << lane) - 1ull))] = (unsigned short)k;
        n_out += __builtin_popcountll(bits);
    }
    if (lane == 0) meta->nalive[b] = (unsigned)n_out;
}
#endif

#ifdef SDFK_CELLS
// rows of row block rb plus the cell of brick (rb, window c) and that cell's sphere (wave-uniform; scalar loads)
static __device__ __forceinline__ void sdfk_brick_cell(const sdfk_rowgeom& g, const sdfk_cells& cl, unsigned rb, unsigned c,
                                                       long long& r0, long long& rend, uint2& span, float4& S) {
    unsigned slot, blk;
    sdfk_block_rows(g, rb, r0, rend, &slot, &blk);
    const unsigned sx = slot == 0xffffffffu ? 0u : cl.lv.xoff + slot;
    const unsigned cell = ((sx >> cl.lv.lx) * cl.lv.ncy + (blk >> cl.lv.ly)) * cl.lv.ncz + (c >> cl.lv.lz);
    S = make_float4(0.0f, 0.0f, 0.0f, -1.0f);
    span = make_uint2(0u, SDFK_ALL_ALIVE);
    // (the launch is padded with bricks beyond the last one: their row block does not exist, and neither does a cell for it)
    if (cl.enabled && r0 < rend && cell < cl.ncells) {
        const uint2 sp = cl.span[cell];
        span = make_uint2(__builtin_amdgcn_readfirstlane(sp.x), __builtin_amdgcn_readfirstlane(sp.y));
        const float4 t = cl.sph[cell];
#ifdef SDFK_FLAT
        S = make_float4(t.x, t.z, t.y, t.w);                   // (the registers of phase A hold (x, z, y))
#else
        S = t;
#endif
    }
}
#endif
#if defined(SDFK_CHAIN) && defined(SDFK_CELLS)
// The same decision from the CELL's candidate list: one member per lane, evaluated at the brick's centre on the spot (no
// table of leaf values in LDS) — the first 64 stay in a register, longer lists are evaluated a second time for the
// comparison. A brick that is not inside its cell's sphere, or whose cell has no list, takes every member.
// `sp` (the cell's span) and `first` (this lane's entry of the first batch) were loaded BEFORE the coordinates were waited
// for, so the only memory round trip left between the bounds and the decision is the members' parameters.
static __device__ __forceinline__ void sdfk_chain_fold_cells(sdfk_rowmeta* meta, int b, int lane, const sdfk_cells& cl, uint2 sp,
                                                             unsigned first, const float* __restrict__ PRM,
                                                             const float* __restrict__ TAB) {
    const float4 cc = meta->bound[b];
    const V3T<float> ctr = {cc.x, cc.y, cc.z};
    const float rho = cc.w, cmag = 1e-6f * (fabsf(cc.x) + fabsf(cc.y) + fabsf(cc.z) + rho);
    unsigned off = 0u, cnt = SDFK_NLEAF;
    bool listed = false;
    if (cl.enabled && __builtin_amdgcn_readfirstlane(meta->inside[b]) != 0u && sp.y != SDFK_ALL_ALIVE) {
        off = sp.x; cnt = sp.y; listed = true;
    }
    float m = 3.0e38f, e0 = 3.0e38f;
    unsigned r0 = 0u;
#pragma unroll 1
    for (unsigned j0 = 0u; j0 < cnt; j0 += 64u) {
        const unsigned j = j0 + (unsigned)lane;
        const bool in = j < cnt;
        unsigned rec = 0u;
        if (in) rec = listed ? (j0 == 0u ? first : cl.cand[off + j]) : sdfk_member_record(j);
        float e = 3.0e38f;
        if (in) e = SDFK_CHAIN_SGN * sdfk_leaf_rec<float>(rec, ctr, PRM, TAB);
        if (j0 == 0u) { e0 = e; r0 = rec; }
        m = fminf(m, e);
    }
#pragma unroll
    for (int o = 1; o < 64; o <<= 1) m = fminf(m, __shfl_xor(m, o));
    const float thr0 = 1.0001f * SDFK_CHAIN_KMAX * rho + SDFK_CHAIN_KMAX * cmag + 1e-6f * (1.0f + fabsf(m));
    unsigned n_out = 0u;
#pragma unroll 1
    for (unsigned j0 = 0u; j0 < cnt; j0 += 64u) {
        const unsigned j = j0 + (unsigned)lane;
        const bool in = j < cnt;
        unsigned rec = r0;
        float e = e0;
        if (j0 != 0u) {
            rec = in ? (listed ? cl.cand[off + j] : sdfk_member_record(j)) : 0u;
            e = 3.0e38f;
            if (in) e = SDFK_CHAIN_SGN * sdfk_leaf_rec<float>(rec, ctr, PRM, TAB);
        }
        const bool run = in && !(e - m >= thr0 + 1e-6f * fabsf(e));
        const unsigned long long bits = __ballot(run);
        const unsigned pos = n_out + (unsigned)__builtin_popcountll(bits & ((1ull << lane) - 1ull));
        if (run && pos < SDFK_ALIST_CAP) meta->alist[b][pos] = rec;
        n_out += (unsigned)__builtin_popcountll(bits);
    }
    // more survivors than the list in LDS holds (dense scenes): the brick runs its cell's whole candidate list straight from
    // memory — a superset in the chain's order — and every member only where there is no such list
    if (lane == 0) {
        meta->nalive[b] = n_out <= SDFK_ALIST_CAP ? n_out : (listed ? SDFK_LIST_ALIVE : SDFK_ALL_ALIVE);
        meta->aspan[b] = make_uint2(off, cnt);
    }
}
#endif

// phases A and B of the tile of this workgroup; returns this wave's first brick (row block, window)
#ifdef SDFK_CELLS
#define SDFK_CELLS_PARAM , const sdfk_cells& cl
#define SDFK_CELLS_PASS , cl
#else
#define SDFK_CELLS_PARAM
#define SDFK_CELLS_PASS
#endif
template <typename SRC>
static __device__ __forceinline__ void sdfk_rows_prepare(const float* __restrict__ PRM, const float* __restrict__ TAB,
                                                         const SRC& s, const sdfk_rowgeom& g, sdfk_rowmeta* meta,
                                                         unsigned tile, unsigned& rb0, unsigned& c0 SDFK_CELLS_PARAM) {
    const int lane = sdfk_tx() & 63, wave = __builtin_amdgcn_readfirstlane(sdfk_tx() >> 6);
    const unsigned q0 = tile * SDFK_RNBRICK + wave * SDFK_RWBRICKS;            // first brick of this wave
    rb0 = sdfk_udiv(q0, g.nchunk, g.inv_nchunk);                // (back in an SGPR: what is derived from it stays scalar)
    c0 = q0 - rb0 * g.nchunk;
    unsigned rb = rb0, c = c0;
#if SDFK_RWBRICKS <= 2 && !defined(SDFK_NOHOIST)
    // two-wave workgroups on the north-star grid; with four bricks per wave the registers this takes cost more)
    sdfk_rowregs hregs[SDFK_RWBRICKS];
    bool live[SDFK_RWBRICKS];
#ifdef SDFK_CELLS
    uint2 cspan[SDFK_RWBRICKS];
    unsigned cfirst[SDFK_RWBRICKS];
    float4 csph[SDFK_RWBRICKS];
#endif
#pragma unroll
    for (int j = 0; j < SDFK_RWBRICKS; ++j) {
        long long r0, rend;
#ifdef SDFK_CELLS
        sdfk_brick_cell(g, cl, rb, c, r0, rend, cspan[j], csph[j]);
        cfirst[j] = 0u;                                          // the lane's entry of the list's first batch: in flight with the coordinates
        if (cspan[j].y != SDFK_ALL_ALIVE && (unsigned)lane < cspan[j].y) cfirst[j] = cl.cand[cspan[j].x + (unsigned)lane];
#else
        sdfk_block_rows(g, rb, r0, rend);
#endif
        live[j] = q0 + j < g.nbricks && r0 < rend;               // (blocks of the last plane beyond the slab: nothing)
        if (live[j]) sdfk_rows_load(s, g, r0, rend, c, lane, hregs[j]);
        if (++c == g.nchunk) { c = 0; ++rb; }
    }
#pragma unroll
    for (int j = 0; j < SDFK_RWBRICKS; ++j)
#ifdef SDFK_CELLS
        if (live[j]) sdfk_rows_bounds(hregs[j], lane, meta, wave * SDFK_RWBRICKS + j, csph[j]);
#else
        if (live[j]) sdfk_rows_bounds(hregs[j], lane, meta, wave * SDFK_RWBRICKS + j);
#endif
        else if (lane == 0) { meta->bound[wave * SDFK_RWBRICKS + j] = make_float4(0.0f, 0.0f, 0.0f, 1.0f); meta->uniform[wave * SDFK_RWBRICKS + j] = 0u; }   // (masks: never read)
#else
#ifdef SDFK_CELLS
    bool live[SDFK_RWBRICKS];
    uint2 cspan[SDFK_RWBRICKS];
    unsigned cfirst[SDFK_RWBRICKS];
#endif
#pragma unroll
    for (int j = 0; j < SDFK_RWBRICKS; ++j) {
        long long r0, rend;
#ifdef SDFK_CELLS
        float4 csph;
        sdfk_brick_cell(g, cl, rb, c, r0, rend, cspan[j], csph);
        cfirst[j] = 0u;
        if (cspan[j].y != SDFK_ALL_ALIVE && (unsigned)lane < cspan[j].y) cfirst[j] = cl.cand[cspan[j].x + (unsigned)lane];
        live[j] = q0 + j < g.nbricks && r0 < rend;
#else
        sdfk_block_rows(g, rb, r0, rend);
#endif
#ifdef SDFK_ABLATE_EDGE
        if (q0 + j < g.nbricks && r0 < rend && sdfk_interior(g.L, c)) {
#else
        if (q0 + j < g.nbricks && r0 < rend) {
#endif
            sdfk_rowregs regs;
            sdfk_rows_load(s, g, r0, rend, c, lane, regs);
#ifdef SDFK_CELLS
            sdfk_rows_bounds(regs, lane, meta, wave * SDFK_RWBRICKS + j, csph);
#else
            sdfk_rows_bounds(regs, lane, meta, wave * SDFK_RWBRICKS + j);
#endif
        } else if (lane == 0) {                                   // a dead brick still meets a probe lane: harmless values
            meta->bound[wave * SDFK_RWBRICKS + j] = make_float4(0.0f, 0.0f, 0.0f, 1.0f);
            meta->uniform[wave * SDFK_RWBRICKS + j] = 0u;
        }
        if (++c == g.nchunk) { c = 0; ++rb; }
    }
#endif
    __syncthreads();
#if defined(SDFK_CHAIN) && defined(SDFK_CELLS)
    // every wave folds ITS bricks from their cells' lists: nothing crosses waves any more (no probe centres, no table of
    // leaf values, two barriers fewer than the path below)
#pragma unroll
    for (int j = 0; j < SDFK_RWBRICKS; ++j) {
// ... 199 lines not shown
                    const unsigned rec = __builtin_amdgcn_readfirstlane(SDFK_AREC(i));
                    f2 val[SDFK_NP];
                    SDFK_EACH val[q] = sdfk_leaf_rec<f2>(rec, P[q], PRM, TAB);
                    if (i == 0u) { SDFK_EACH acc[q] = val[q]; }
                    else { SDFK_EACH acc[q] = SDFK_CHAIN_CMB(acc[q], val[q], PRM); }
                }
            }
#if SDFK_CHAIN_STAGED
            else
#pragma unroll 1
            for (unsigned c0 = 0; c0 < cnt; c0 += SDFK_CHUNK) {
                const unsigned nc = cnt - c0 < SDFK_CHUNK ? cnt - c0 : SDFK_CHUNK;
                __builtin_amdgcn_fence(__ATOMIC_RELEASE, "wavefront");      // (the previous chunk has been read)
                __builtin_amdgcn_wave_barrier();
#pragma unroll 1
                for (unsigned it = (unsigned)lane; it < nc * SDFK_NPLMAX; it += 64u) {
                    const unsigned ch = it / SDFK_NPLMAX, w = it - ch * SDFK_NPLMAX;
                    const unsigned rec = SDFK_AREC(c0 + ch);
                    const unsigned at = (rec & 0xffffffu) + w;
                    meta.cprm[b][ch][w] = PRM[at < SDFK_NPARAMS ? at : SDFK_NPARAMS - 1u];
                    if (w == 0u) meta.cgrp[b][ch] = rec >> 24;
                }
                __builtin_amdgcn_fence(__ATOMIC_RELEASE, "wavefront");
                __builtin_amdgcn_wave_barrier();
                __builtin_amdgcn_fence(__ATOMIC_ACQUIRE, "wavefront");
#pragma unroll 1
                for (unsigned i = 0; i < nc; ++i) {
                    const unsigned grp = __builtin_amdgcn_readfirstlane(meta.cgrp[b][i]);
                    const float* cp = &meta.cprm[b][i][0];
                    f2 val[SDFK_NP];
                    SDFK_EACH val[q] = sdfk_leaf_at<f2>(grp, P[q], cp, TAB);
                    if (c0 + i == 0u) { SDFK_EACH acc[q] = val[q]; }
                    else { SDFK_EACH acc[q] = SDFK_CHAIN_CMB(acc[q], val[q], PRM); }
                }
            }
#endif
            SDFK_EACH res[q] = sdfk_chain_tail<f2>(acc[q], P[q], PRM, TAB);
#if defined(SDFK_DEBUG_NALIVE) && defined(SDFK_CELLS)
            // test aid: instead of the field, how the brick ran — survivors on its list; 100000 + entries when it ran its cell's
            // whole list (more survivors than SDFK_ALIST_CAP); -1 when it ran every member
            SDFK_EACH res[q] = sp<f2>(all_alive ? -1.0f : (list_alive ? 100000.0f + (float)cnt : (float)cnt));
#endif
        }
#endif
#ifdef SDFK_FLAGS                                                  // (the flag-writing build) one bit per point instead of the field
        {
            // BRICK-TILED layout: the word of (row r, window k) is flags[(brick * 16 + r % 16)], so the 64 lanes of the
            // wave — lane = 4 * row + octet of the window — write the brick's 64 bytes as ONE contiguous store, and every
            // (row, window) slot belongs to one brick, also where two rows share a flat window: no atomics (a linear bit
            // string needs an atomic OR in the edge windows and 16 partial-line stores per brick). The compaction
            unsigned bits = 0u;
            SDFK_EACH bits |= ((sdfk_sel_key(res[q].x) <= thr ? 1u : 0u) | (sdfk_sel_key(res[q].y) <= thr ? 2u : 0u)) << (2 * q);
            if (!interior) {                                       // an edge window: only the points of this row
                unsigned ok = 0u;
                SDFK_EACH {
                    if (z + 2 * q >= 0 && z + 2 * q <= last) ok |= 1u << (2 * q);
                    if (z + 2 * q + 1 >= 0 && z + 2 * q + 1 <= last) ok |= 2u << (2 * q);
                }
                bits &= ok;
            }
            if (!live_row) bits = 0u;                              // rows past the end of the last block: empty slots
            reinterpret_cast<unsigned char*>(flags)[(unsigned long long)(q0 + j) * 64ull + (unsigned)lane] = (unsigned char)bits;
        }
#else
        if (live_row) {
            float* po = out + f;
            if (interior) {
#pragma unroll
                for (int q = 0; q < SDFK_NP; q += 2) {
                    sdfk_f4u v = {res[q].x, res[q].y, res[q + 1].x, res[q + 1].y};
                    __builtin_nontemporal_store(v, reinterpret_cast<sdfk_f4u*>(po + 2 * q));
                }
            } else {
                SDFK_EACH {
                    if (z + 2 * q >= 0 && z + 2 * q <= last) po[2 * q] = res[q].x;
                    if (z + 2 * q + 1 >= 0 && z + 2 * q + 1 <= last) po[2 * q + 1] = res[q].y;
                }
            }
        }
#endif
    }
  }
}
#ifdef SDFK_WPE
#define SDFK_ROWS_ATTR __attribute__((amdgpu_waves_per_eu(SDFK_WPE, SDFK_WPE)))
#else
#define SDFK_ROWS_ATTR
#endif
#ifdef SDFK_CELLS
#define SDFK_CELLS_KARG , sdfk_cells cl
// ---- the pre-pass: one WAVE per cell ------------------------------------------------------------------------------
struct sdfk_cellpass {
    sdfk_celllevel lv, parent;                  // parent.ncx == 0: no coarser level — the candidates are all members
    float4* __restrict__ sph;                   // this level's cells: sphere ...
    uint2* __restrict__ span;                   // ... and list
    const float4* __restrict__ psph;            // the parent level's
    const uint2* __restrict__ pspan;
    unsigned* __restrict__ cand;                // the pool (records: sdfk_member_record)
    unsigned* __restrict__ head;                // this level's SDFK_POOL_SHARDS allocation heads, 64 bytes apart
    unsigned base, shard_cap;                   // shard h owns entries [base + h * shard_cap, base + (h + 1) * shard_cap)
    unsigned ncells, pad0;
    float inflate, pad;                         // factor on the radius the LIST is computed for (coarse level: > 1, see below)
};
// point z of local row `row`
static __device__ __forceinline__ float3 sdfk_cell_point(const SrcArray& s, const sdfk_rowgeom& g, long long row, unsigned z) {
    const float* p = s.co + row * (long long)g.L + z;
#ifdef SDFK_XY
    return make_float3(p[0], p[s.stride], 0.0f);
#else
    return make_float3(p[0], p[s.stride], p[2 * s.stride]);
#endif
}
static __device__ __forceinline__ float3 sdfk_cell_point(const SrcGrid& s, const sdfk_rowgeom& g, long long row, unsigned z) {
    const unsigned long long g0 = (unsigned long long)(g.row0 + row);
    if (g.yrows) return make_float3(s.ax0[g0], s.ax1[z], s.ax2[0]);
    const unsigned long long ix = g0 / s.n1;
    return make_float3(s.ax0[ix], s.ax1[(unsigned)(g0 - ix * s.n1)], s.ax2[z]);
}
// rows [r0, rend) and blocks of plane slot sl of a level (slot 0 = the leading partial plane when lv.xoff > 0)
static __device__ __forceinline__ bool sdfk_slot_rows(const sdfk_rowgeom& g, const sdfk_celllevel& lv, unsigned sl, long long& r0,
                                                      long long& rend) {
    if (lv.xoff > 0u && sl == 0u) { r0 = 0; rend = g.seg0; return g.seg0 > 0u; }
    if (sl < lv.xoff) return false;
    r0 = (long long)g.seg0 + (long long)(sl - lv.xoff) * g.prow;
    rend = r0 + g.prow < g.R ? r0 + g.prow : g.R;
    return r0 < g.R;
}
template <typename SRC>
static __device__ __forceinline__ void sdfk_cells_kernel(const float* __restrict__ PRM, const float* __restrict__ TAB, const SRC& s,
                                                         const sdfk_rowgeom& g, const sdfk_cellpass& cp) {
    const int lane = sdfk_tx() & 63;
    const unsigned cell = __builtin_amdgcn_readfirstlane(sdfk_bx() * 4u + (sdfk_tx() >> 6));
    if (cell >= cp.ncells) return;
    const sdfk_celllevel lv = cp.lv;
    const unsigned cz = cell % lv.ncz, t0 = cell / lv.ncz, cy = t0 % lv.ncy, cx = t0 / lv.ncy;
    // what the cell covers in index space: slots [sA, sB], blocks [b0, b1], points [zlo, zhi] of a row
    const unsigned sA = cx << lv.lx;
    unsigned sB = ((cx + 1u) << lv.lx) - 1u;
    long long ra0, ra1, rb0, rb1;
    bool some = sdfk_slot_rows(g, lv, sA, ra0, ra1);
    if (lv.xoff > 0u && cx == 0u) sB = 0u;
    while (some && sB > sA && !sdfk_slot_rows(g, lv, sB, rb0, rb1)) --sB;
    if (sB == sA) { rb0 = ra0; rb1 = ra1; }
    const long long lo = (long long)(cy << lv.ly) * SDFK_RROWS, hi = (long long)((cy + 1u) << lv.ly) * SDFK_RROWS;
    some = some && ra0 + lo < ra1;
    const unsigned w0 = cz << lv.lz, w1 = ((cz + 1u) << lv.lz) < g.nchunk ? ((cz + 1u) << lv.lz) - 1u : g.nchunk - 1u;
    some = some && w0 < g.nchunk;
    if (!some) {                                                // no brick maps here
        if (lane == 0) { cp.sph[cell] = make_float4(0.0f, 0.0f, 0.0f, -1.0f); cp.span[cell] = make_uint2(0u, 0u); }
        return;
    }
    // windows are aligned in the FLAT array: window k of a row starts up to 31 points before point 32 k of that row
    const unsigned zlo = 32u * w0 > 31u ? 32u * w0 - 31u : 0u;
    const unsigned zhi = 32u * w1 + 31u < g.L ? 32u * w1 + 31u : g.L - 1u;
    // the eight corner points (a lattice cell is their convex hull): lanes 0..7
    const long long rowsel[4] = {ra0 + lo, (ra0 + hi < ra1 ? ra0 + hi : ra1) - 1, (rb0 + lo < rb1 ? rb0 + lo : rb1 - 1),
                                 (rb0 + hi < rb1 ? rb0 + hi : rb1) - 1};
    const float3 pt = sdfk_cell_point(s, g, rowsel[(lane >> 1) & 3], (lane & 1) ? zhi : zlo);
    float mnx = pt.x, mxx = pt.x, mny = pt.y, mxy = pt.y, mnz = pt.z, mxz = pt.z;
#pragma unroll
    for (int o = 1; o < 8; o <<= 1) {
        mnx = fminf(mnx, __shfl_xor(mnx, o)); mxx = fmaxf(mxx, __shfl_xor(mxx, o));
        mny = fminf(mny, __shfl_xor(mny, o)); mxy = fmaxf(mxy, __shfl_xor(mxy, o));
        mnz = fminf(mnz, __shfl_xor(mnz, o)); mxz = fmaxf(mxz, __shfl_xor(mxz, o));
    }
    const V3T<float> ctr = {0.5f * (mnx + mxx), 0.5f * (mny + mxy), 0.5f * (mnz + mxz)};
// ... 50 lines not shown
#pragma unroll 4
    for (unsigned j0 = 64u * SDFK_CELL_NB; j0 < cnt; j0 += 64u) {
        const unsigned j = j0 + (unsigned)lane;
        if (j < cnt) m = fminf(m, SDFK_CHAIN_SGN * sdfk_leaf_rec<float>(listed ? cp.cand[off + j] : sdfk_member_record(j), c, PRM, TAB));
    }
#pragma unroll
    for (int o = 1; o < 64; o <<= 1) m = fminf(m, __shfl_xor(m, o));
    const float thr0 = 1.0001f * SDFK_CHAIN_KMAX * rho + SDFK_CHAIN_KMAX * cmag + 1e-6f * (1.0f + fabsf(m));
    unsigned total = 0u;
#pragma unroll
    for (int bt = 0; bt < SDFK_CELL_NB; ++bt)
        if (64u * bt < cnt) total += (unsigned)__builtin_popcountll(__ballot(64u * bt + (unsigned)lane < cnt && !(ev[bt] - m >= thr0 + 1e-6f * fabsf(ev[bt]))));
#pragma unroll 4
    for (unsigned j0 = 64u * SDFK_CELL_NB; j0 < cnt; j0 += 64u) {
        const unsigned j = j0 + (unsigned)lane;
        bool run = false;
        if (j < cnt) {
            const float e = SDFK_CHAIN_SGN * sdfk_leaf_rec<float>(listed ? cp.cand[off + j] : sdfk_member_record(j), c, PRM, TAB);
            run = !(e - m >= thr0 + 1e-6f * fabsf(e));
        }
        total += (unsigned)__builtin_popcountll(__ballot(run));
    }
    // per microsecond and address), so the pool is cut into SDFK_POOL_SHARDS shards with a head each, dealt by cell index
    unsigned at = 0u;
    const unsigned shard = cell & (SDFK_POOL_SHARDS - 1u);
    if (lane == 0) at = atomicAdd(cp.head + 16u * shard, total);
    at = __shfl(at, 0);
    if (at > cp.shard_cap || total > cp.shard_cap - at) {       // the shard is full: bricks of this cell probe every member
        if (lane == 0) cp.span[cell] = make_uint2(0u, SDFK_ALL_ALIVE);
        return;
    }
    at += cp.base + shard * cp.shard_cap;
    unsigned n_out = 0u;
#pragma unroll
    for (int bt = 0; bt < SDFK_CELL_NB; ++bt)
        if (64u * bt < cnt) {
            const bool run = 64u * bt + (unsigned)lane < cnt && !(ev[bt] - m >= thr0 + 1e-6f * fabsf(ev[bt]));
            const unsigned long long bits = __ballot(run);
            if (run) cp.cand[at + n_out + (unsigned)__builtin_popcountll(bits & ((1ull << lane) - 1ull))] = rv[bt];
            n_out += (unsigned)__builtin_popcountll(bits);
        }
#pragma unroll 4
    for (unsigned j0 = 64u * SDFK_CELL_NB; j0 < cnt; j0 += 64u) {
        const unsigned j = j0 + (unsigned)lane;
        bool run = false;
        unsigned rec = 0u;
        if (j < cnt) {
            rec = listed ? cp.cand[off + j] : sdfk_member_record(j);
            const float e = SDFK_CHAIN_SGN * sdfk_leaf_rec<float>(rec, c, PRM, TAB);
            run = !(e - m >= thr0 + 1e-6f * fabsf(e));
        }
        const unsigned long long bits = __ballot(run);
        if (run) cp.cand[at + n_out + (unsigned)__builtin_popcountll(bits & ((1ull << lane) - 1ull))] = rec;
        n_out += (unsigned)__builtin_popcountll(bits);
    }
    if (lane == 0) cp.span[cell] = make_uint2(at, total);
}
#else
#define SDFK_CELLS_KARG
#endif
)SDFKR";
static const char kRowsArray[] = R"SDFKR(
extern "C" __global__ __launch_bounds__(64 * SDFK_RWAVES) SDFK_ROWS_ATTR void sdfk_spec_r(
    const float* __restrict__ PRM, const float* __restrict__ TAB, const float* __restrict__ co, long long stride,
    sdfk_rowgeom g, float* __restrict__ out, unsigned* __restrict__ flags, unsigned thr SDFK_CELLS_KARG) {
    const SrcArray s = {co, stride};
    sdfk_rows_kernel(PRM, TAB, s, g, out, flags, thr SDFK_CELLS_PASS);
}
#ifdef SDFK_CELLS
extern "C" __global__ __launch_bounds__(256) void sdfk_spec_cells(
    const float* __restrict__ PRM, const float* __restrict__ TAB, const float* __restrict__ co, long long stride,
    sdfk_rowgeom g, sdfk_cellpass cp) {
    const SrcArray s = {co, stride};
    sdfk_cells_kernel(PRM, TAB, s, g, cp);
}
#endif
)SDFKR";
static const char kRowsGrid[] = R"SDFKR(
// the same on a regular grid expanded from three per-axis tables (no coordinate array: 4 B/point); the slab
// starts at a row boundary and out[0] is its first point
extern "C" __global__ __launch_bounds__(64 * SDFK_RWAVES) void sdfk_spec_rg(
    const float* __restrict__ PRM, const float* __restrict__ TAB, SrcGrid s, sdfk_rowgeom g, float* __restrict__ out,
    unsigned* __restrict__ flags, unsigned thr SDFK_CELLS_KARG) {
    sdfk_rows_kernel(PRM, TAB, s, g, out, flags, thr SDFK_CELLS_PASS);
}
#ifdef SDFK_CELLS
extern "C" __global__ __launch_bounds__(256) void sdfk_spec_cellsg(
    const float* __restrict__ PRM, const float* __restrict__ TAB, SrcGrid s, sdfk_rowgeom g, sdfk_cellpass cp) {
    sdfk_cells_kernel(PRM, TAB, s, g, cp);
}
#endif
)SDFKR";
static const char kRowsMask[] = R"SDFKR(
// test aid: the skip masks (two 64-bit words per brick: sites 0-31, 32-63; bit 2k = first operand of site k
// skipped, bit 2k+1 = second) followed by the "uniform rows" flag in a third word
extern "C" __global__ __launch_bounds__(64 * SDFK_RWAVES) void sdfk_spec_rmask(
    const float* __restrict__ PRM, const float* __restrict__ TAB, const float* __restrict__ co, long long stride,
    sdfk_rowgeom g, unsigned long long* __restrict__ masks) {
    __shared__ __attribute__((aligned(16))) sdfk_rowmeta meta;
    const SrcArray s = {co, stride};
    unsigned rb, c;
    sdfk_rows_prepare(PRM, TAB, s, g, &meta, sdfk_bx(), rb, c);
    const unsigned q = sdfk_bx() * SDFK_RNBRICK + sdfk_tx();
    if (sdfk_tx() < SDFK_RNBRICK && q < g.nbricks) {
        masks[3ull * q] = meta.mask[0][sdfk_tx()];
        masks[3ull * q + 1] = meta.mask[1][sdfk_tx()];
        masks[3ull * q + 2] = meta.uniform[sdfk_tx()];
    }
}
)SDFKR";

namespace {

struct Gen {
    const sdfk_opinfo* ops;
    int n_ops;
    const uint32_t* code;
    size_t n_instr;
    const std::vector<sdfk_cullsite>* sites;
    std::string s;
    bool rows = false;

    std::vector<int> root_slot;
    int n_root = 0;
    void find_roots() {
        root_slot.assign(n_instr, -1);
        bool c0_intact = true;
        for (size_t i = 0; i < n_instr; ++i) {
            const uint32_t w = code[2 * i];
            const unsigned op = w & 255u, a = (w >> 8) & 255u, b = (w >> 16) & 255u;
            if ((int)op >= n_ops) continue;
            if (ops[op].kind != SDFK_KIND_C_C) continue;
            if (!strcmp(ops[op].name, "XFORM") && b == 0 && c0_intact && n_root < 64) root_slot[i] = n_root++;
            if (a == 0) c0_intact = false;
        }
    }

    void instr_x(size_t i, const char* indent, int mode) {
        const int r = root_slot.empty() ? -1 : root_slot[i];
        if (r < 0 || mode == 0 || (rows && mode == 1)) {
            instr(i, indent, rows && mode == 2);
            return;
        }
        char buf[1400];
        const uint32_t w = code[2 * i], poff = code[2 * i + 1];
        const unsigned a = (w >> 8) & 255u;
        if (rows) {
            snprintf(buf, sizeof buf,
                     "%sif constexpr (ZRUN) {\n"
                     "#ifdef SDFK_FLAT\n"
                     "%s  const V3T<float> bs = op_xform_base_x(X, PRM + %u);\n"
                     "%s  const V3P bp = {sp<f2>(bs.x), sp<f2>(bs.y), sp<f2>(bs.z)};\n"
                     "%s  SDFK_EACH C_%u[q] = op_xform_y(bp, C_0[q].y, PRM + %u);\n"
                     "#else\n"
                     "%s  const V3T<float> bs = op_xform_base(X, Y, PRM + %u);\n"
                     "%s  const V3P bp = {sp<f2>(bs.x), sp<f2>(bs.y), sp<f2>(bs.z)};\n"
                     "%s  SDFK_EACH C_%u[q] = op_xform_z(bp, C_0[q].z, PRM + %u);\n"
                     "#endif\n"
                     "%s} else { SDFK_EACH C_%u[q] = op_xform(C_0[q], PRM + %u, TAB, 0); }\n",
                     indent, indent, poff, indent, indent, a, poff, indent, poff, indent, indent, a, poff, indent, a, poff);
        } else if (mode == 1) {
            snprintf(buf, sizeof buf,
                     "%s{ const V3T<float> bs = op_xform_base(C_0.x, C_0.y, PRM + %u); bases[%d] = bs.x; bases[%d] = bs.y; "
                     "bases[%d] = bs.z;\n%s  C_%u = op_xform_z(bs, C_0.z, PRM + %u); }\n",
                     indent, poff, 3 * r, 3 * r + 1, 3 * r + 2, indent, a, poff);
        } else {
            snprintf(buf, sizeof buf,
// ... 767 lines not shown
        if (!ours && t.comb >= g.chain_sites.front().a0 && t.comb <= g.chain_sites.back().comb) return false;
    }
    const std::vector<sdfk_cullsite>* keep = g.sites;
    g.sites = &g.chain_sites;
    g.region_lo = g.chain_sites.front().a0;
    g.region_hi = g.chain_sites.back().comb;
    bool ok = g.analyse_leaves() && g.analyse_chain(result_reg) && g.leaves_contiguous();
    if (ok && g.groups.size() > 255) ok = false;
    for (size_t k = 0; ok && k < g.leaves.size(); ++k)
        if (g.leaves[k].hi - g.leaves[k].lo + 1 > 256) ok = false;
    if (!ok) {
        g.sites = keep;
        g.region_lo = 0;
        g.region_hi = (size_t)-1;
    }
    return ok;
}
int sdfk_chain_mode(const sdfk_opinfo* ops, int n_ops, const uint32_t* code, size_t n_instr, int result_reg,
                    const std::vector<sdfk_cullsite>& sites_all) {
    Gen g{ops, n_ops, code, n_instr, &sites_all, std::string()};
    return chain_analyse(g, result_reg, &sites_all) ? (int)g.leaves.size() : 0;
}

std::string sdfk_generate_source(const sdfk_opinfo* ops, int n_ops, const uint32_t* code, size_t n_instr,
                                 int result_reg, const std::vector<sdfk_cullsite>& sites, int flavour,
                                 const std::vector<sdfk_cullsite>* sites_all) {
    const bool all = flavour == SDFK_FL_ALL;
    const bool plain = all || flavour == SDFK_FL_PLAIN_ARRAY || flavour == SDFK_FL_PLAIN_GRID;
    const bool tile = !sites.empty() && (all || flavour == SDFK_FL_TILE_ARRAY || flavour == SDFK_FL_TILE_GRID ||
                                         flavour == SDFK_FL_TILE_MASK);
    const bool flat = flavour == SDFK_FL_ROWS2D_ARRAY || flavour == SDFK_FL_ROWS2D_GRID;
    const bool rowk = !sites.empty() && (all || flat || flavour == SDFK_FL_ROWS_ARRAY || flavour == SDFK_FL_ROWS_GRID ||
                                         flavour == SDFK_FL_ROWS_MASK);
    Gen g{ops, n_ops, code, n_instr, &sites, std::string()};
    g.s.reserve(sizeof(kEmbeddedDevice) + sizeof(kEmbeddedAccess) + sizeof(kWrappers) + sizeof(kTileKernel) +
                sizeof(kRowsKernel) + 800 * n_instr + 4096);
    g.s += kEmbeddedDevice;
    g.s += "\n";
    g.s += kEmbeddedAccess;
    char buf[64];
    if (flavour == SDFK_FL_RAYS || flavour == SDFK_FL_OCCUPANCY) {
        bool chain = false;
        if (chain_analyse(g, result_reg, sites_all)) {
            g.emit_chain_common();
            chain = true;
        } else {
            g.s += "\ntemplate <typename T> static __device__ __forceinline__ T sdfk_point(V3T<T> C_0, "
                   "const float* __restrict__ PRM, const float* __restrict__ TAB, const float* __restrict__ AUX, "
                   "long long AUXS) {\n";
            g.declare("V3T<T>", "T", false);
            for (size_t i = 0; i < n_instr; ++i) g.instr(i, "    ");
            snprintf(buf, sizeof buf, "    return V_%d;\n}\n", result_reg);
            g.s += buf;
        }
        if (flavour == SDFK_FL_OCCUPANCY) {
            g.s += kEmbeddedOccdev;
            g.s += kSpecField;
            g.s += kOccupancy;
            return g.s;
        }
        g.s += kEmbeddedRaydev;
        g.s += kSpecField;
        g.s += kRays;
        if (chain) {
            g.s += "\n#ifndef SDFK_RAYS_CULL_MIN_LEAVES\n#define SDFK_RAYS_CULL_MIN_LEAVES 64    // (measured: DESIGN 4.14 has the table)\n#endif\n"
                   "#if SDFK_NLEAF >= SDFK_RAYS_CULL_MIN_LEAVES\n";
            g.s += kWaveHelpers;
            g.s += kRaysCull;
            g.s += "#endif\n";
        }
        return g.s;
    }
    if (chain_analyse(g, result_reg, sites_all)) {
        const bool flat2 = flavour == SDFK_FL_ROWS2D_ARRAY || flavour == SDFK_FL_ROWS2D_GRID;
        g.emit_chain_common();
        if (plain) {
            g.s += kWrappers;
            if (all || flavour == SDFK_FL_PLAIN_ARRAY) g.s += kWrappersArray;
            if (all || flavour == SDFK_FL_PLAIN_GRID) g.s += kWrappersGrid;
        }
        if (all || flat2 || flavour == SDFK_FL_ROWS_ARRAY || flavour == SDFK_FL_ROWS_GRID || flavour == SDFK_FL_ROWS_MASK) {
            g.s += kWaveHelpers;
            if (flat2) g.s += "\n#define SDFK_FLAT 1\n";
            g.s += "\n#define SDFK_NP 4\n#define SDFK_EACH _Pragma(\"unroll\") for (int q = 0; q < SDFK_NP; ++q)\n"
                   "#define SDFK_NMASK 2\n"
                   "#define SDFK_SIMT 1\n#define SDFK_NSUB 1\n"
                   "#ifndef SDFK_CELLS_MIN_LEAVES\n#define SDFK_CELLS_MIN_LEAVES 64\n#endif\n"
                   "#if !defined(SDFK_NO_CELLS) && SDFK_NLEAF > SDFK_CELLS_MIN_LEAVES\n#define SDFK_CELLS 1\n#endif\n"
                   "#ifndef SDFK_LEAF_UNROLL\n#define SDFK_LEAF_UNROLL _Pragma(\"unroll 4\")\n#endif\n";
            g.s += kSimtGeometry;
            g.emit_probe_leaves(g.leaves.size() >= 128, true);
            g.s += kRowsKernel;
            if (all || flavour == SDFK_FL_ROWS_ARRAY || flavour == SDFK_FL_ROWS2D_ARRAY) g.s += kRowsArray;
            if (all || flavour == SDFK_FL_ROWS_GRID || flavour == SDFK_FL_ROWS2D_GRID) g.s += kRowsGrid;
        }
        return g.s;
    }
    if (plain) {
        g.s += "\ntemplate <typename T> static __device__ __forceinline__ T sdfk_point(V3T<T> C_0, "
               "const float* __restrict__ PRM, const float* __restrict__ TAB, const float* __restrict__ AUX, "
               "long long AUXS) {\n";
        g.declare("V3T<T>", "T", false);
        for (size_t i = 0; i < n_instr; ++i) g.instr(i, "    ");
        snprintf(buf, sizeof buf, "    return V_%d;\n}\n", result_reg);
        g.s += buf;
        g.s += kWrappers;
        if (all || flavour == SDFK_FL_PLAIN_ARRAY) g.s += kWrappersArray;
        if (all || flavour == SDFK_FL_PLAIN_GRID) g.s += kWrappersGrid;
    }
    if (tile || rowk) g.s += kWaveHelpers;
    if (tile) {
        std::vector<size_t> order(sites.size());
        for (size_t i = 0; i < order.size(); ++i) order[i] = i;
        std::stable_sort(order.begin(), order.end(), [&](size_t x, size_t y) {
            return sites[x].comb - sites[x].a0 > sites[y].comb - sites[y].a0;
        });
        order.resize(std::min<size_t>(order.size(), 31));
        std::sort(order.begin(), order.end());
        std::vector<sdfk_cullsite> flat;
        for (size_t i : order) flat.push_back(sites[i]);
        g.sites = &flat;
        g.find_roots();
        snprintf(buf, sizeof buf, "\n#define SDFK_NROOT %d\n", g.n_root > 0 ? g.n_root : 1);
        g.s += buf;
        g.emit_probe();
        g.emit_culled(result_reg);
        g.s += kTileKernel;
        if (all || flavour == SDFK_FL_TILE_ARRAY) g.s += kTileArray;
        if (all || flavour == SDFK_FL_TILE_GRID) g.s += kTileGrid;
        if (all || flavour == SDFK_FL_TILE_MASK) g.s += kTileMask;
        g.sites = &sites;
    }
    if (rowk) {
        g.rows = true;
        g.root_slot.clear();
        g.n_root = 0;
        g.find_roots();
        if (flat) g.s += "\n#define SDFK_FLAT 1\n";
        g.s += "\n#define SDFK_NP 4\n#define SDFK_EACH _Pragma(\"unroll\") for (int q = 0; q < SDFK_NP; ++q)\n";
        {
            char nm[64];
            snprintf(nm, sizeof nm, "#define SDFK_NMASK %zu\n", std::max<size_t>(2, (sites.size() + 31) / 32));
            g.s += nm;
        }
        g.s += "#ifndef SDFK_CHAIN_LOOP_MIN\n#define SDFK_CHAIN_LOOP_MIN 100000   // chains of at least this many sites run as a loop over the levels that survive\n#endif\n"
               "// the even bits of x, packed into the low 32 bits (wave-uniform: scalar unit)\n"
               "static __device__ __forceinline__ unsigned long long sdfk_even_bits(unsigned long long x) {\n"
               "    x &= 0x5555555555555555ull;\n"
               "    x = (x | (x >> 1)) & 0x3333333333333333ull;\n"
               "    x = (x | (x >> 2)) & 0x0f0f0f0f0f0f0f0full;\n"
               "    x = (x | (x >> 4)) & 0x00ff00ff00ff00ffull;\n"
               "    x = (x | (x >> 8)) & 0x0000ffff0000ffffull;\n"
               "    x = (x | (x >> 16)) & 0x00000000ffffffffull;\n"
               "    return x;\n}\n";
        g.simt = g.analyse_leaves();
        if (g.simt) {
            char def[160];
            snprintf(def, sizeof def, "\n#ifndef SDFK_NOSIMT\n#define SDFK_SIMT 1\n#endif\n#define SDFK_NLEAF %zu\n", g.leaves.size());
            g.s += def;
            g.s += kSimtGeometry;
            g.emit_groups();
            g.emit_probe_leaves();
            g.emit_probe_fold();
        }
        g.emit_probe();
        g.emit_rows_culled(result_reg);
        g.s += kRowsKernel;
        if (all || flavour == SDFK_FL_ROWS_ARRAY || flavour == SDFK_FL_ROWS2D_ARRAY) g.s += kRowsArray;
        if (all || flavour == SDFK_FL_ROWS_GRID || flavour == SDFK_FL_ROWS2D_GRID) g.s += kRowsGrid;
        if (all || flavour == SDFK_FL_ROWS_MASK) g.s += kRowsMask;
    }
    return g.s;
}
```

include/sdfk.h:

```cpp
#ifndef SDFK_H
#define SDFK_H

#include <stddef.h>
#include <stdint.h>

#ifdef __cplusplus
extern "C" {
#endif

#define SDFK_ABI_VERSION 1

#define SDFK_MODE_AUTO 0
#define SDFK_MODE_INTERPRET 1
#define SDFK_MODE_SPECIALIZED 2
#define SDFK_MODE_NOCULL 3

typedef struct sdfk_program sdfk_program;

int sdfk_abi_version(void);
int sdfk_device_count(void);
const char* sdfk_last_error(void);

sdfk_program* sdfk_program_create(const uint32_t* code, size_t n_instr, const float* params, size_t n_params,
                                  const float* tables, size_t n_tables, int result_reg);
void sdfk_program_destroy(sdfk_program* prog);
int sdfk_program_set_params(sdfk_program* prog, const float* params, size_t n_params);
int sdfk_program_set_cull(sdfk_program* prog, const uint32_t* sites, size_t n_sites, const float* k);
int sdfk_program_chain_members(const sdfk_program* prog);
const char* sdfk_program_source(sdfk_program* prog);
int sdfk_program_compile_check(sdfk_program* prog, size_t* code_size);
#define SDFK_FLAVOUR_PLAIN_ARRAY 0
#define SDFK_FLAVOUR_PLAIN_GRID 1
#define SDFK_FLAVOUR_TILE_ARRAY 2
#define SDFK_FLAVOUR_TILE_GRID 3
#define SDFK_FLAVOUR_TILE_MASK 4
#define SDFK_FLAVOUR_ROWS_ARRAY 5
#define SDFK_FLAVOUR_ROWS_GRID 6
#define SDFK_FLAVOUR_ROWS_MASK 7
#define SDFK_FLAVOUR_ROWS2D_ARRAY 8
#define SDFK_FLAVOUR_ROWS2D_GRID 9
#define SDFK_FLAVOUR_RAYS 10
#define SDFK_FLAVOUR_OCCUPANCY 11
#define SDFK_FLAVOUR_FLAGS 0x100
#define SDFK_FLAVOUR_XY 0x200
int sdfk_program_compile_flavour(sdfk_program* prog, int flavour, size_t* code_size, double* seconds);
void sdfk_debug_cells_stats(int enable, long long* out8);
void sdfk_debug_rays_stats(int enable, long long* out8);
int sdfk_debug_compile_external(sdfk_program* prog, int flavour, size_t* code_size);
void sdfk_jit_drain(void);
void sdfk_jit_cancel(void);
void sdfk_debug_jit_stats(int64_t* builds, double* seconds);
void sdfk_debug_set_rtc_defs(const char* defs);

int sdfk_eval_device(sdfk_program* prog, const float* d_co, int64_t n, int64_t row_stride, float* d_out,
                     void* stream, int mode);
int sdfk_eval_device_rows(sdfk_program* prog, const float* d_co, int64_t n, int64_t row_stride, int64_t row_len,
                          float* d_out, void* stream, int mode);
int sdfk_eval_device_rows3d(sdfk_program* prog, const float* d_co, int64_t n, int64_t row_stride, int64_t row_len,
                            int64_t plane_rows, int64_t first_row_in_plane, float* d_out, void* stream, int mode);
int sdfk_eval_device_rows2d(sdfk_program* prog, const float* d_co, int64_t n, int64_t row_stride, int64_t row_len,
                            float* d_out, void* stream, int mode);
int sdfk_eval_device_rows2d_xy(sdfk_program* prog, const float* d_xy, int64_t n, int64_t row_stride, int64_t row_len,
                               float* d_out, void* stream, int mode);
int sdfk_eval_host(sdfk_program* prog, const void* co, int co_dtype, int64_t n, int64_t row_stride, float* out,
                   int device, int mode);
int sdfk_eval_host_resident(sdfk_program* prog, const void* co, int co_dtype, int64_t n, int64_t row_stride,
                            float* d_out, int device, int mode);
int sdfk_eval_grid(sdfk_program* prog, const float* ax0, int64_t n0, const float* ax1, int64_t n1, const float* ax2,
                   int64_t n2, int64_t start, int64_t count, float* d_out, void* stream, int mode);
int sdfk_eval_grid_host(sdfk_program* prog, const float* ax0, int64_t n0, const float* ax1, int64_t n1,
                        const float* ax2, int64_t n2, int64_t start, int64_t count, float* out, int device, int mode);
int sdfk_eval_grid_sharded(sdfk_program* prog, const float* ax0, int64_t n0, const float* ax1, int64_t n1,
                           const float* ax2, int64_t n2, int n_shards, const int* devices, float* out, int mode);
int sdfk_eval_grid_sharded_device(sdfk_program* prog, const float* ax0, int64_t n0, const float* ax1, int64_t n1,
                                  const float* ax2, int64_t n2, int n_shards, const int* devices, int gather_device,
                                  float* d_full, int mode);
void sdfk_set_default_mode(int mode);
int sdfk_debug_brick_masks(sdfk_program* prog, const float* d_co, int64_t n, int64_t row_stride, uint64_t* d_masks,
                           void* stream);
int sdfk_debug_row_masks(sdfk_program* prog, const float* d_co, int64_t n, int64_t row_stride, int64_t row_len,
                         uint64_t* d_masks, int64_t* n_bricks, int* brick_rows, void* stream);

int sdfk_eval_device_aux(sdfk_program* prog, const float* d_co, int64_t n, int64_t row_stride, const float* d_aux,
                         int n_aux, int64_t aux_stride, float* d_out, void* stream, int mode);
int sdfk_eval_grid_aux(sdfk_program* prog, const float* ax0, int64_t n0, const float* ax1, int64_t n1, const float* ax2,
                       int64_t n2, int64_t start, int64_t count, const float* d_aux, int n_aux, int64_t aux_stride,
                       float* d_out, void* stream, int mode);
int sdfk_field_min(const float* d_field, int64_t n, float* out_min, void* stream);
int sdfk_grid_box_average(float* d_field, int64_t n0, int64_t n1, int64_t n2, int k0, int k1, int k2, int iterations,
                          void* d_scratch, void* stream);
int sdfk_grid_edge_detect(float* d_field, int64_t n0, int64_t n1, int64_t n2, void* d_scratch, void* stream);
int sdfk_grid_signed(float* d_field, int64_t n0, int64_t n1, int64_t n2, float sep_min, int crop, void* d_scratch,
                     void* stream);
int sdfk_debug_box_variant(int64_t n0, int64_t n1, int64_t n2, int k0, int k1, int k2, int* out8);
int sdfk_grid_boundary_mask(const float* d_field, int64_t n, float sep_min, unsigned char* d_mask, void* stream);
int sdfk_grid_signed_slab(float* d_slab, int64_t plane0, int64_t planes, const unsigned char* d_mask, int64_t n0, int64_t n1,
                          int64_t n2, int crop, void* d_scratch, void* stream);

size_t sdfk_field_select_scratch(int64_t n);
int sdfk_field_select_finish(int64_t n, int64_t count, int64_t* d_index, int64_t capacity, void* d_scratch, void* stream);

size_t sdfk_eval_select_scratch(int64_t n, int64_t row_len);
int sdfk_eval_device_select(sdfk_program* prog, const float* d_co, int64_t n, int64_t row_stride, int64_t row_len, int flat,
                            float threshold, int64_t* d_index, int64_t capacity, int64_t* count, void* d_scratch,
                            void* stream, int mode);
int sdfk_eval_grid_select(sdfk_program* prog, const float* ax0, int64_t n0, const float* ax1, int64_t n1, const float* ax2,
                          int64_t n2, int64_t start, int64_t count_points, float threshold, int64_t* d_index,
                          int64_t capacity, int64_t* count, void* d_scratch, void* stream, int mode);
int sdfk_eval_select_finish(sdfk_program* prog, int64_t n, int64_t row_len, int mode, int64_t count, int64_t* d_index,
                            int64_t capacity, void* d_scratch, void* stream);
int sdfk_field_select(const float* d_field, int64_t n, float threshold, int64_t* d_index, int64_t capacity,
                      int64_t* count, void* d_scratch, void* stream);
int sdfk_field_gradient(const float* d_field, int64_t n0, int64_t n1, int64_t n2, int ncomp, int normalize,
                        float* d_vec, int64_t row_stride, void* stream);

int sdfk_field_crossings_2d(const float* d_uu, const float* d_ww, int64_t n0, int64_t n1, int64_t n2, double w, double d,
                            double thr, signed char* d_sign, void* stream);
int sdfk_lcwg_eval(int variant, const float* d_uu, const float* d_ww, int64_t n0, int64_t n1, int64_t n2, double w, double d,
                   int sign_kind, double sign_value, const void* d_sign, float* d_vec, int64_t row_stride, void* stream);
int sdfk_lcwg_old_eval(int variant, const float* d_r, int64_t r_stride, const float* d_uu, int64_t n, double w, double d,
                       float* d_vec, int64_t row_stride, void* stream);

typedef struct {
    int32_t op;
    int32_t src[2];
    float imm[4];
} sdfk_vec_instr;
int sdfk_vec_eval_device(const sdfk_vec_instr* prog, int n_instr, const float* d_p, int64_t n, int64_t p_stride,
                         const float* d_streams, int n_streams, int64_t stream_stride, int out_kind, float* d_out,
                         int64_t out_stride, void* stream);
void sdfk_vec_set_interpret(int on);
const char* sdfk_vec_source(const sdfk_vec_instr* prog, int n_instr, int n_streams, int out_kind);
int sdfk_vec_compile_check(const sdfk_vec_instr* prog, int n_instr, int n_streams, int out_kind, size_t* code_size);
int sdfk_vec_eval_host(const sdfk_vec_instr* prog, int n_instr, const void* p, int p_dtype, int64_t n, const float* ax0,
                       int64_t n0, const float* ax1, int64_t n1, const float* ax2, int64_t n2, const float* streams,
                       int n_streams, int out_kind, float* out, int device);

int sdfk_linspace_f32(double lo, double hi, int64_t n, float* out);
int64_t sdfk_point_tree_build(const float* pts, int64_t m, int leaf, float* table, int64_t table_cap, int64_t* order,
                              int64_t* n_root, int64_t* point_base);

int sdfk_grid_fill(float* d_co, int64_t row_stride, const float* ax0, int64_t n0, const float* ax1, int64_t n1,
                   const float* ax2, int64_t n2, int64_t start, int64_t count, void* stream);

int sdfk_set_device(int device);
void* sdfk_malloc(size_t bytes);
int sdfk_free(void* d_ptr);
int sdfk_memcpy_h2d(void* d_dst, const void* src, size_t bytes);
int sdfk_memcpy_d2h(void* dst, const void* d_src, size_t bytes);
int sdfk_memcpy_d2d(void* d_dst, const void* d_src, size_t bytes);
int sdfk_sync(void* stream);
void* sdfk_event_create(void);
int sdfk_event_destroy(void* ev);
int sdfk_event_record(void* ev, void* stream);
int sdfk_event_elapsed_ms(void* ev_start, void* ev_stop, float* ms);
int sdfk_stream_probe(const float* d_co, int64_t n, int64_t row_stride, float* d_out, void* stream);


int sdfk_dual_has_rule(int op);
int sdfk_program_jvp_check(sdfk_program* prog, int* first_bad_op);
// ... 74 lines not shown
```

Baseline: 361,500.

## Add dedicated axis-table grid row kernel and cache device axis tables

Adds a separate row-block kernel for grid sources in which each lane loads the coordinates it evaluates directly from the axis tables and keeps them in registers. This removes LDS staging of z windows and one barrier, and computes sub-brick bounds within the wave. Row indices are split into (ix, iy) with a host-computed reciprocal instead of a division. sdfk_eval_grid also caches the uploaded axis tables per device and drops its trailing stream synchronize. The cost is more code paths, a persistent cache compared with memcmp on every call, and a separate kernel skeleton to keep correct.

Result: no change. 361,600 (median of 3 runs) (+0.0%).

```diff
diff --git a/aegolius_amd/_engine.py b/aegolius_amd/_engine.py
--- a/aegolius_amd/_engine.py
+++ b/aegolius_amd/_engine.py
@@ -81,6 +81,7 @@
     "sdfk_eval_grid_host": (_int, [_vp, _vp, _i64, _vp, _i64, _vp, _i64, _i64, _i64, _vp, _int, _int]),
     "sdfk_set_default_mode": (None, [_int]),
     "sdfk_debug_brick_masks": (_int, [_vp, _vp, _i64, _i64, _vp, _vp]),
+    "sdfk_debug_grid_row": (_int, [_c.c_uint32, _c.c_uint32, _c.POINTER(_c.c_uint32), _c.POINTER(_c.c_uint32)]),
     "sdfk_linspace_f32": (_int, [_c.c_double, _c.c_double, _i64, _vp]),
     "sdfk_point_tree_build": (_i64, [_vp, _i64, _int, _vp, _i64, _vp, _vp, _vp]),
     "sdfk_grid_fill": (_int, [_vp, _i64, _vp, _i64, _vp, _i64, _vp, _i64, _i64, _i64, _vp]),
diff --git a/aegolius_amd/csrc/sdfk.hip b/aegolius_amd/csrc/sdfk.hip
--- a/aegolius_amd/csrc/sdfk.hip
+++ b/aegolius_amd/csrc/sdfk.hip
@@ -580,7 +580,12 @@
     int yrows;
     unsigned prow, seg0, nb0, bpp;
     unsigned inv_nchunk, inv_bpp;
+    unsigned inv_n1;
 };
+static_assert(sizeof(RowGeom) == 64, "sdfk_rowgeom of the generated source: the array kernels' argument layout");
+static unsigned sdfk_rowdiv_inv(unsigned long long d) {
+    return (unsigned)std::min<unsigned long long>(0xffffffffull, (1ull << 32) / (d ? d : 1ull));
+}
 static bool rows_geometry(long long n, long long row_len, RowGeom* g, long long plane_rows = 0, long long plane_phase = 0,
                           bool planes_on = false) {
     if (row_len < 32 || row_len > 0x7fffffffLL || n <= 0 || n % row_len != 0) return false;
@@ -610,6 +615,7 @@
     g->bpp = (unsigned)bpp;
     g->inv_nchunk = (unsigned)std::min<unsigned long long>(0xffffffffull, (1ull << 32) / (unsigned long long)nchunk);
     g->inv_bpp = (unsigned)std::min<unsigned long long>(0xffffffffull, (1ull << 32) / (unsigned long long)bpp);
+    g->inv_n1 = 0;
     return true;
 }
 static int tile_threads() { return 64 * tile_waves(); }
@@ -1536,6 +1542,7 @@
                 SrcGrid g = *grid;
                 rg.row0 = grid->start / grow;
                 rg.yrows = grid->n2 > 1 ? 0 : 1;
+                rg.inv_n1 = sdfk_rowdiv_inv(grid->n1);
                 if (with_cells) {
                     void* src[] = {&g};
                     rc = prepare_cells(p, d, sk->fn[1], rg, src, 1, prm, tab, stream, &cells);
@@ -1784,18 +1791,69 @@
     return 0;
 }
 
+struct CachedAxes {
+    std::vector<float> host;
+    int64_t n0 = 0, n1 = 0, n2 = 0;
+    AxisTables dev;
+};
+static std::mutex g_axes_mutex;
+static std::map<int, std::shared_ptr<CachedAxes>>& g_axes_cache = *new std::map<int, std::shared_ptr<CachedAxes>>;
+static int cached_axes(const float* ax0, int64_t n0, const float* ax1, int64_t n1, const float* ax2, int64_t n2,
+                       hipStream_t stream, std::shared_ptr<CachedAxes>* out, SrcGrid* g, int64_t start) {
+    if (!ax0 || !ax1 || !ax2 || n0 < 1 || n1 < 1 || n2 < 1) return fail(-1, "grid axes missing or empty");
+    if (n1 > 0x7fffffff || n2 > 0x7fffffff) return fail(-1, "grid axis too long");
+    int device = 0;
+    HIPCHK(hipGetDevice(&device));
+    std::shared_ptr<CachedAxes> c;
+    {
+        std::lock_guard<std::mutex> lock(g_axes_mutex);
+        auto it = g_axes_cache.find(device);
+        if (it != g_axes_cache.end()) c = it->second;
+    }
+    const bool hit = c && c->n0 == n0 && c->n1 == n1 && c->n2 == n2 &&
+                     memcmp(c->host.data(), ax0, (size_t)n0 * sizeof(float)) == 0 &&
+                     memcmp(c->host.data() + n0, ax1, (size_t)n1 * sizeof(float)) == 0 &&
+                     memcmp(c->host.data() + n0 + n1, ax2, (size_t)n2 * sizeof(float)) == 0;
+    if (!hit) {
+        c = std::make_shared<CachedAxes>();
+        c->n0 = n0; c->n1 = n1; c->n2 = n2;
+        c->host.resize((size_t)(n0 + n1 + n2));
+        memcpy(c->host.data(), ax0, (size_t)n0 * sizeof(float));
+        memcpy(c->host.data() + n0, ax1, (size_t)n1 * sizeof(float));
+        memcpy(c->host.data() + n0 + n1, ax2, (size_t)n2 * sizeof(float));
+        HIPCHK(hipMalloc(&c->dev.d, c->host.size() * sizeof(float)));
+        HIPCHK(hipMemcpyAsync(c->dev.d, c->host.data(), c->host.size() * sizeof(float), hipMemcpyHostToDevice, stream));
+        HIPCHK(hipStreamSynchronize(stream));
+        std::lock_guard<std::mutex> lock(g_axes_mutex);
+        g_axes_cache[device] = c;
+    }
+    g->ax0 = c->dev.d;
+    g->ax1 = c->dev.d + n0;
+    g->ax2 = c->dev.d + n0 + n1;
+    g->n1 = (unsigned)n1;
+    g->n2 = (unsigned)n2;
+    g->start = start;
+    *out = c;
+    return 0;
+}
+
 extern "C" int sdfk_eval_grid(sdfk_program* p, const float* ax0, int64_t n0, const float* ax1, int64_t n1,
                               const float* ax2, int64_t n2, int64_t start, int64_t count, float* d_out, void* stream,
                               int mode) {
     if (!d_out) return fail(-1, "sdfk_eval_grid: null output");
     if (start < 0 || count < 0 || start + count > n0 * n1 * n2) return fail(-1, "sdfk_eval_grid: range outside the grid");
-    AxisTables t;
+    std::shared_ptr<CachedAxes> t;
     SrcGrid g;
-    int rc = upload_axes(ax0, n0, ax1, n1, ax2, n2, (hipStream_t)stream, &t, &g, start);
+    int rc = cached_axes(ax0, n0, ax1, n1, ax2, n2, (hipStream_t)stream, &t, &g, start);
     if (rc) return rc;
-    rc = run(p, nullptr, &g, count, d_out, stream, mode, aligned16(d_out));
-    if (rc) return rc;
-    HIPCHK(hipStreamSynchronize((hipStream_t)stream));
+    return run(p, nullptr, &g, count, d_out, stream, mode, aligned16(d_out));
+}
+
+extern "C" int sdfk_debug_grid_row(uint32_t row, uint32_t n1, uint32_t* ix, uint32_t* iy) {
+    if (!ix || !iy || n1 < 1) return fail(-1, "sdfk_debug_grid_row: bad arguments");
+    const unsigned q = sdfk_rowdiv(row, n1, sdfk_rowdiv_inv(n1));
+    *ix = q;
+    *iy = row - q * n1;
     return 0;
 }
 
@@ -1906,6 +1964,7 @@
                 int r = 0;
                 if (!d_slab && hipMalloc(&d_slab, (size_t)count * sizeof(float)) != hipSuccess) r = fail(-5, "out of device memory for the slab");
                 if (r == 0) r = sdfk_eval_grid(p, ax0, n0, ax1, n1, ax2, n2, start, count, d_slab, stream, mode);
+                if (r == 0 && in_place && hipStreamSynchronize(stream) != hipSuccess) r = fail(-6, "evaluation of the slab failed");
                 if (r == 0 && !in_place) {
                     if (hipMemcpyPeerAsync(d_full + start, gather_device, d_slab, dev, (size_t)count * sizeof(float), stream) != hipSuccess ||
                         hipStreamSynchronize(stream) != hipSuccess)
diff --git a/aegolius_amd/csrc/sdfk_access.h b/aegolius_amd/csrc/sdfk_access.h
--- a/aegolius_amd/csrc/sdfk_access.h
+++ b/aegolius_amd/csrc/sdfk_access.h
@@ -14,6 +14,12 @@
     unsigned n1, n2;
     long long start;
 };
+
+static __host__ __device__ __forceinline__ unsigned sdfk_rowdiv(unsigned a, unsigned d, unsigned inv) {
+    unsigned q = (unsigned)(((unsigned long long)a * inv) >> 32);
+    while (a - q * d >= d) ++q;
+    return q;
+}
 
 typedef float sdfk_f4 __attribute__((ext_vector_type(4)));
 static __device__ __forceinline__ float4 sdfk_stream_load4(const float* p) {
diff --git a/aegolius_amd/csrc/sdfk_codegen.cpp b/aegolius_amd/csrc/sdfk_codegen.cpp
--- a/aegolius_amd/csrc/sdfk_codegen.cpp
+++ b/aegolius_amd/csrc/sdfk_codegen.cpp
@@ -661,6 +661,13 @@
                                                  // 4096: 2.21 -> 2.11 (SDFK_STAGE_MIN=64 against 2); -DSDFK_CHAIN_STAGED=1 brings it back
 static_assert(SDFK_NP == 2 || SDFK_NP == 4, "2 or 4 packed pairs per lane");
 static_assert(SDFK_RNBRICK <= 64 * SDFK_RWAVES, "one probe lane per brick");
+// Builds that only hold the axis-table entry point (SDFK_GRIDSRC, set by the generator) take a skeleton of their own,
+// sdfk_rowsg_kernel below: coordinates straight from the tables in the evaluation layout, nothing staged. The text up
+// to there is then left out; -DSDFK_GRID_LEGACY keeps it. Candidate-list builds (SDFK_CELLS) stay on the shared skeleton.
+#if defined(SDFK_GRIDSRC) && !defined(SDFK_GRID_LEGACY) && !defined(SDFK_CELLS) && !SDFK_CHAIN_STAGED && SDFK_NP == 4 && \
+    (!defined(SDFK_SIMT) || SDFK_NSUB <= 8)
+#define SDFK_GRID_BLOCKS 1
+#endif
 
 typedef float sdfk_f4u __attribute__((ext_vector_type(4), aligned(4)));
 
@@ -672,7 +679,9 @@
 #define SDFK_LIST_ALIVE 0xfffffffeu
 #endif
 struct sdfk_rowmeta {
+#ifndef SDFK_GRID_BLOCKS
     float z[SDFK_RNBRICK][SDFK_RBRICK];         // [row of the brick][point of the window]
+#endif
     float2 xy[SDFK_RNBRICK][SDFK_RROWS];
     float4 bound[SDFK_RNBRICK];
     unsigned long long mask[SDFK_NMASK][SDFK_RNBRICK];   // two bits per site: SDFK_NMASK x 32 sites (2 words up to 64 sites)
@@ -707,6 +716,7 @@
     unsigned prow, seg0, nb0, bpp;              // planes of prow rows after a first partial plane of seg0 rows (nb0 blocks);
                                                 // bpp blocks per plane: a block never holds rows of two planes
     unsigned inv_nchunk, inv_bpp;               // floor(2^32 / nchunk), floor(2^32 / bpp): divisions as one v_mul_hi
+    unsigned inv_n1;                            // grid flavour: floor(2^32 / n1) (sdfk_rowdiv); fills the struct's tail padding
 };
 #ifdef SDFK_CELLS
 // Candidate lists (chain mode). The bricks are grouped into CELLS in index space — 2^lx plane slots x 2^ly row blocks x
@@ -782,6 +792,7 @@
     return make_float4(rowp[min(max(z, 0), last)], rowp[min(max(z + 1, 0), last)], rowp[min(max(z + 2, 0), last)],
                        rowp[min(max(z + 3, 0), last)]);
 }
+#ifndef SDFK_GRID_BLOCKS
 // the 4 points [z, z+4) of row `row` (row = r0 + dr, r0 wave-uniform) as three quads
 static __device__ __forceinline__ void sdfk_rows_fetch(const SrcArray& s, const sdfk_rowgeom& g, long long r0, int dr, int z,
                                                        bool interior, float4& X, float4& Y, float4& Z) {
@@ -814,6 +825,7 @@
     Y = make_float4(y, y, y, y);
     Z = sdfk_win_quad(s.ax2, z, (int)g.L - 1, interior);
 }
+#endif
 static __device__ __forceinline__ float sdfk_prev_lane(float v) {   // value of lane-1 within a row of 16 lanes
     return __builtin_bit_cast(float, __builtin_amdgcn_update_dpp(__builtin_bit_cast(int, v), __builtin_bit_cast(int, v), 0x111, 0xf, 0xf, false));
 }
@@ -825,6 +837,7 @@
     return (int)(f - rl);
 }
 
+#ifndef SDFK_GRID_BLOCKS
 // phase A, part 1: issue the loads of one brick (wave-uniform r0, k); 8 rows x 32 points per instruction
 struct sdfk_rowregs {
     float4 X[SDFK_RLOADS], Y[SDFK_RLOADS], Z[SDFK_RLOADS];
@@ -998,6 +1011,7 @@
 }
 #endif
 
+#endif   // !SDFK_GRID_BLOCKS
 #if defined(SDFK_CHAIN) && !defined(SDFK_CELLS)
 // Chain mode, one WAVE per brick: which children run on this brick, from the leaf values at its centre. A hard min (max:
 // signs flipped, e_k = +-d_k) is exact, associative and commutative, so the ORDER of the chain does not matter for a
@@ -1126,6 +1140,7 @@
 #define SDFK_CELLS_PARAM
 #define SDFK_CELLS_PASS
 #endif
+#ifndef SDFK_GRID_BLOCKS
 template <typename SRC>
 static __device__ __forceinline__ void sdfk_rows_prepare(const float* __restrict__ PRM, const float* __restrict__ TAB,
                                                          const SRC& s, const sdfk_rowgeom& g, sdfk_rowmeta* meta,
@@ -1491,6 +1506,392 @@
     }
   }
 }
+#endif   // !SDFK_GRID_BLOCKS
+#ifdef SDFK_GRID_BLOCKS
+// ---- row blocks on axis tables ---------------------------------------------------------------------------------------
+// The same windows, tiles and stores as above, but a lane reads what it evaluates: lane = 4 * row + octet owns 8 consecutive
+// points of ONE row from phase A on. The two coordinates its row shares come as two table reads, its 8 values of the third
+// one straight from that axis' table (two 16-byte reads in interior windows, clamped single reads in edge windows), and
+// they stay in registers until phase C. Every row segment has one x and one y by construction, so nothing is compared
+// (flat grids: z = ax2[0] must still be exactly 0 for the shared transform, a scalar test). A sub-brick of the probe is
+// 8 or 16 rows of one octet = one value per lane, so centre and radius are computed in the wave, with the expressions of
+// sdfk_sub_centre / sdfk_rows_bounds (maxima are exact: the order they are taken in does not show), and written to the
+// probe's centres directly: no staging in LDS, no pass of one wave over rows x points, one barrier fewer.
+static_assert(SDFK_RLPR == 4 && SDFK_RROWS == 16 && SDFK_RZ / 4 == 2 * SDFK_NP, "a lane's points are one sub-brick's share of its row");
+struct sdfk_gbrick {
+    f2 w[SDFK_NP];                              // the coordinate that varies along the row (z; flat grids: y)
+    float x, y;                                 // the two the row shares (x, y; flat grids: x, z)
+};
+// (ix, iy) of global row g0 (wave-uniform): 32-bit arithmetic with the host's reciprocal; from 2^32 rows on, shift and
+// subtract — no division instruction sequence either way
+static __device__ __forceinline__ void sdfk_grid_row(const SrcGrid& s, const sdfk_rowgeom& g, unsigned long long g0,
+                                                     unsigned long long& ix, unsigned& iy) {
+    if ((g0 >> 32) == 0ull) {
+        const unsigned a = (unsigned)g0;
+        const unsigned q = __builtin_amdgcn_readfirstlane(sdfk_rowdiv(a, s.n1, g.inv_n1));
+        ix = q;
+        iy = a - q * s.n1;
+    } else {
+        unsigned long long q = 0ull, r = g0;
+#pragma unroll 1
+        for (int b = 63; b >= 0; --b)
+            if ((r >> b) >= (unsigned long long)s.n1) { r -= (unsigned long long)s.n1 << b; q |= 1ull << b; }
+        ix = q;
+        iy = (unsigned)r;
+    }
+}
+// phase A, part 1: this lane's share of one brick (wave-uniform r0, rend, k)
+static __device__ __forceinline__ void sdfk_gbrick_load(const SrcGrid& s, const sdfk_rowgeom& g, long long r0, long long rend,
+                                                        unsigned k, int lane, sdfk_gbrick& B) {
+    const int lr = lane / SDFK_RLPR, zq = (lane % SDFK_RLPR) * (2 * SDFK_NP);
+    const int dr = r0 + lr < rend ? lr : (int)(rend - 1 - r0);       // rows past the end of the block: its last row again
+    long long f;
+    const int z = sdfk_win_z(r0 + dr, g.L, k, zq, &f);
+    const unsigned long long g0 = (unsigned long long)(g.row0 + r0);
+#ifdef SDFK_FLAT                                                      // (x, y, z) = (ax0[row], ax1[point], ax2[0])
+    const float* __restrict__ tab = s.ax1;
+    B.x = s.ax0[g0 + (unsigned)dr];
+    B.y = s.ax2[0];
+#else
+    const float* __restrict__ tab = s.ax2;
+    unsigned long long ix;
+    unsigned iy;
+    sdfk_grid_row(s, g, g0, ix, iy);
+    iy += (unsigned)dr;
+    while (iy >= s.n1) { iy -= s.n1; ++ix; }                         // a block may cross planes
+    B.x = s.ax0[ix];
+    B.y = s.ax1[iy];
+#endif
+    if (sdfk_interior(g.L, k)) {
+#pragma unroll
+        for (int q = 0; q < SDFK_NP; q += 2) {
+            const sdfk_f4u v = *reinterpret_cast<const sdfk_f4u*>(tab + z + 2 * q);
+            B.w[q] = {v.x, v.y};
+            B.w[q + 1] = {v.z, v.w};
+        }
+    } else {                                                          // edge window: the nearest point of the row, branch-free
+        const int last = (int)g.L - 1;
+        SDFK_EACH B.w[q] = {tab[min(max(z + 2 * q, 0), last)], tab[min(max(z + 2 * q + 1, 0), last)]};
+    }
+}
+static __device__ __forceinline__ float sdfk_gshfl(float v, int l) {
+    return __builtin_bit_cast(float, __builtin_amdgcn_ds_bpermute(l << 2, __builtin_bit_cast(int, v)));
+}
+static __device__ __forceinline__ float sdfk_gxor_max(float v, int o) {
+    return sd_rawmax(v, __builtin_bit_cast(float, __builtin_amdgcn_ds_bpermute(((int)(sdfk_tx() & 63) ^ o) << 2, __builtin_bit_cast(int, v))));
+}
+// phase A, part 2: bounding spheres of brick b, written where the probe reads them
+// (uniform: wave-uniform — the shared transform of phase C applies; always true on 3-D grids)
+static __device__ __forceinline__ void sdfk_gbrick_bounds(const sdfk_gbrick& B, int lane, sdfk_rowmeta* meta, int b, bool uniform) {
+#ifdef SDFK_SIMT
+    if (lane == 0) {
+#pragma unroll
+        for (int w = 0; w < SDFK_NMASK; ++w) meta->mask[w][b] = ~0ull;   // the fold lanes AND their decisions into these
+    }
+#endif
+#ifdef SDFK_ABLATE_BOUNDS
+    if (lane == 0) meta->bound[b] = make_float4(0.f, 0.f, 0.f, 1.f);
+#ifdef SDFK_SIMT
+    if (lane < SDFK_NSUB) meta->cen[b * SDFK_NSUB + lane] = make_float4(0.f, 0.f, 0.f, 1.f);
+#endif
+    return;
+#endif
+#if defined(SDFK_SIMT) && SDFK_NSUB > 1
+    if (uniform) {
+        // sub-brick = rows [ra, re) x this lane's octet. 8 centres: two row parts, split in the middle — or, where the
+        // brick's rows come from two planes, where x changes: each part then lies in one plane and is bounded tightly
+        constexpr int NZP = 4, NRP = SDFK_NSUB / NZP;
+        const int lr = lane / SDFK_RLPR, zp = lane % SDFK_RLPR;
+        int s = SDFK_RROWS / NRP;
+        if (NRP == 2) {
+            const unsigned x0 = __builtin_amdgcn_readlane(__builtin_bit_cast(unsigned, B.x), 0);
+            const unsigned x1 = __builtin_amdgcn_readlane(__builtin_bit_cast(unsigned, B.x), 63);
+            if (x0 != x1) s = (int)(__builtin_ctzll(__ballot(__builtin_bit_cast(unsigned, B.x) != x0)) >> 2);
+        }
+        const bool hi = NRP == 2 && lr >= s;
+        const int ra = hi ? s : 0, re = (NRP == 2 && !hi) ? s : SDFK_RROWS;
+        const float xa = sdfk_gshfl(B.x, ra * SDFK_RLPR), xe = sdfk_gshfl(B.x, (re - 1) * SDFK_RLPR);
+        const float ya = sdfk_gshfl(B.y, ra * SDFK_RLPR), ye = sdfk_gshfl(B.y, (re - 1) * SDFK_RLPR);
+        const float za = sdfk_gshfl(B.w[0].x, ra * SDFK_RLPR + zp), ze = sdfk_gshfl(B.w[SDFK_NP - 1].y, (re - 1) * SDFK_RLPR + zp);
+        const float cx = 0.5f * (xa + xe), cy = 0.5f * (ya + ye), cz = 0.5f * (za + ze);
+        const float dx = B.x - cx, dy = B.y - cy;
+        float zm = 0.0f;
+        SDFK_EACH zm = sd_rawmax(zm, sd_rawmax(sd_abs(B.w[q].x - cz), sd_abs(B.w[q].y - cz)));
+        const float val = sd_fma(zm, zm, sd_fma(dx, dx, dy * dy));
+        float m0 = hi ? 0.0f : val, m1 = hi ? val : 0.0f;             // (values are >= +0)
+#pragma unroll
+        for (int o = SDFK_RLPR; o < 64; o <<= 1) {
+            m0 = sdfk_gxor_max(m0, o);
+            if (NRP == 2) m1 = sdfk_gxor_max(m1, o);
+        }
+        const float r2 = hi ? m1 : m0;
+        const float rho = 1.00001f * sqrtf(r2) + 1e-30f;
+        if (lr == ra) {
+#ifdef SDFK_FLAT
+            meta->cen[b * SDFK_NSUB + (hi ? NZP : 0) + zp] = make_float4(cx, cz, cy, rho);
+#else
+            meta->cen[b * SDFK_NSUB + (hi ? NZP : 0) + zp] = make_float4(cx, cy, cz, rho);
+#endif
+        }
+        return;
+    }
+#endif
+    // one sphere around the whole brick: midpoint of its first and last point
+    const float cx = 0.5f * (sdfk_lane(B.x, 0) + sdfk_lane(B.x, 63));
+    const float cy = 0.5f * (sdfk_lane(B.y, 0) + sdfk_lane(B.y, 63));
+    const float cz = 0.5f * (sdfk_lane(B.w[0].x, 0) + sdfk_lane(B.w[SDFK_NP - 1].y, 63));
+    float d2 = 0.0f;
+    if (uniform) {                                   // one x, y per row segment: |p - c|^2 = dxy^2 + max |z - cz|^2
+        const float dx = B.x - cx, dy = B.y - cy;
+        float zm = 0.0f;
+        SDFK_EACH zm = sd_rawmax(zm, sd_rawmax(sd_abs(B.w[q].x - cz), sd_abs(B.w[q].y - cz)));
+        d2 = sd_fma(zm, zm, sd_fma(dx, dx, dy * dy));
+    } else {
+        const f2 ax = sp<f2>(B.x) - cx, ay = sp<f2>(B.y) - cy;
+        SDFK_EACH {
+            const f2 az = B.w[q] - cz;
+            const f2 da = sd_fma(ax, ax, sd_fma(ay, ay, az * az));
+            d2 = sd_rawmax(d2, sd_rawmax(da.x, da.y));
+        }
+    }
+    const float r2 = sdfk_wave_max(d2);
+#ifdef SDFK_FLAT
+    const float4 bnd = make_float4(cx, cz, cy, 1.00001f * sqrtf(r2) + 1e-30f);
+#else
+    const float4 bnd = make_float4(cx, cy, cz, 1.00001f * sqrtf(r2) + 1e-30f);
+#endif
+    if (lane == 0) meta->bound[b] = bnd;
+#ifdef SDFK_SIMT
+    if (lane < SDFK_NSUB) meta->cen[b * SDFK_NSUB + lane] = bnd;
+#endif
+}
+static __device__ __forceinline__ bool sdfk_gbrick_uniform(const sdfk_gbrick& B) {     // wave-uniform
+#ifdef SDFK_FLAT
+    // z = 0 exactly (M2 * 0 drops out of every root transform); any other ax2[0]: every point on its own, as above
+    return (__builtin_amdgcn_readfirstlane(__builtin_bit_cast(unsigned, B.y)) & 0x7fffffffu) == 0u;
+#else
+    return true;
+#endif
+}
+// phases A and B of the tile of this workgroup; this wave's first brick (row block, window) and its lanes' coordinates
+static __device__ __forceinline__ void sdfk_rowsg_prepare(const float* __restrict__ PRM, const float* __restrict__ TAB,
+                                                          const SrcGrid& s, const sdfk_rowgeom& g, sdfk_rowmeta* meta,
+                                                          unsigned tile, unsigned& rb0, unsigned& c0,
+                                                          sdfk_gbrick (&B)[SDFK_RWBRICKS]) {
+    const int lane = sdfk_tx() & 63, wave = __builtin_amdgcn_readfirstlane(sdfk_tx() >> 6);
+    const unsigned q0 = tile * SDFK_RNBRICK + wave * SDFK_RWBRICKS;            // first brick of this wave
+    rb0 = sdfk_udiv(q0, g.nchunk, g.inv_nchunk);
+    c0 = q0 - rb0 * g.nchunk;
+    unsigned rb = rb0, c = c0;
+    bool live[SDFK_RWBRICKS];
+#pragma unroll
+    for (int j = 0; j < SDFK_RWBRICKS; ++j) {                    // all of the wave's reads are in flight before the first is used
+        long long r0, rend;
+        sdfk_block_rows(g, rb, r0, rend);
+        live[j] = q0 + j < g.nbricks && r0 < rend;               // (blocks of the last plane beyond the slab: nothing)
+        SDFK_EACH B[j].w[q] = sp<f2>(0.0f);
+        B[j].x = 0.0f;
+        B[j].y = 0.0f;
+        if (live[j]) sdfk_gbrick_load(s, g, r0, rend, c, lane, B[j]);
+        if (++c == g.nchunk) { c = 0; ++rb; }
+    }
+#pragma unroll
+    for (int j = 0; j < SDFK_RWBRICKS; ++j) {
+        const int b = wave * SDFK_RWBRICKS + j;
+        if (live[j]) {
+            sdfk_gbrick_bounds(B[j], lane, meta, b, sdfk_gbrick_uniform(B[j]));
+        } else {                                                  // a dead brick still meets a probe lane: harmless values
+            if (lane == 0) meta->bound[b] = make_float4(0.0f, 0.0f, 0.0f, 1.0f);
+#ifdef SDFK_SIMT
+            if (lane < SDFK_NSUB) meta->cen[b * SDFK_NSUB + lane] = make_float4(0.0f, 0.0f, 0.0f, 1.0f);
+#endif
+        }
+    }
+    __syncthreads();
+#ifdef SDFK_SIMT
+    // lane-parallel probe: every leaf at every centre (all lanes) -> one fold lane per centre ANDs its skip decisions into
+    // the brick's mask (a subtree is skipped only if every sub-brick allows it)
+#ifndef SDFK_ABLATE_PROBE
+    sdfk_probe_leaves(meta->cen, meta->leafval, PRM, TAB);
+    __syncthreads();
+#ifdef SDFK_CHAIN
+#pragma unroll 1
+    for (int j = 0; j < SDFK_RWBRICKS; ++j)
+        if (q0 + j < g.nbricks) sdfk_chain_fold(meta, wave * SDFK_RWBRICKS + j, lane);
+#else
+    if (sdfk_tx() < SDFK_NCEN && tile * SDFK_RNBRICK + sdfk_tx() / SDFK_NSUB < g.nbricks) {
+        const float4 cc = meta->cen[sdfk_tx()];
+        V3T<float> ctr = {cc.x, cc.y, cc.z};
+        unsigned long long mk[SDFK_NMASK];
+        sdfk_probe_fold(meta->leafval, sdfk_tx(), ctr, cc.w, PRM, mk);
+#pragma unroll
+        for (int w = 0; w < SDFK_NMASK; ++w)
+            __hip_atomic_fetch_and(&meta->mask[w][sdfk_tx() / SDFK_NSUB], mk[w], __ATOMIC_RELAXED, __HIP_MEMORY_SCOPE_WORKGROUP);
+    }
+#endif
+#else
+    if (sdfk_tx() < SDFK_RNBRICK) {
+#pragma unroll
+        for (int w = 0; w < SDFK_NMASK; ++w) meta->mask[w][sdfk_tx()] = 0ull;
+    }
+#endif
+#else
+    if (sdfk_tx() < SDFK_RNBRICK && tile * SDFK_RNBRICK + sdfk_tx() < g.nbricks) {
+        const float4 bb = meta->bound[sdfk_tx()];
+        V3T<float> ctr = {bb.x, bb.y, bb.z};
+        unsigned long long mk[SDFK_NMASK];
+#pragma unroll
+        for (int w = 0; w < SDFK_NMASK; ++w) mk[w] = 0ull;
+#if !defined(SDFK_ABLATE_PROBE) && !defined(SDFK_CHAIN)
+        sdfk_probe_r(ctr, bb.w, PRM, TAB, mk);
+#endif
+#pragma unroll
+        for (int w = 0; w < SDFK_NMASK; ++w) meta->mask[w][sdfk_tx()] = mk[w];
+    }
+#endif
+    __syncthreads();
+}
+
+static __device__ __forceinline__ void sdfk_rowsg_kernel(const float* __restrict__ PRM, const float* __restrict__ TAB,
+                                                         const SrcGrid& s, const sdfk_rowgeom& g, float* __restrict__ out,
+                                                         unsigned* __restrict__ flags, unsigned thr) {
+    __shared__ __attribute__((aligned(16))) sdfk_rowmeta meta;
+#ifdef SDFK_LDSPAD
+    if (g.L == 0xffffffffu) meta.pad[sdfk_tx()] = 1.0f;
+#endif
+    const int lane = sdfk_tx() & 63, wave = __builtin_amdgcn_readfirstlane(sdfk_tx() >> 6);
+    const int lr = lane / SDFK_RLPR;
+    const int zq = (lane % SDFK_RLPR) * (2 * SDFK_NP);
+#ifndef SDFK_RTILES
+#define SDFK_RTILES 1
+#endif
+#ifndef SDFK_XGROUP                       // (the runs of tiles per XCD of sdfk_rows_kernel)
+#ifdef SDFK_FLAT
+#define SDFK_XGROUP 4
+#else
+#define SDFK_XGROUP (SDFK_RNBRICK <= 4 ? 16 : (SDFK_RNBRICK <= 8 ? 8 : 4))
+#endif
+#endif
+#pragma unroll 1
+  for (unsigned tt = 0; tt < SDFK_RTILES; ++tt) {
+    const unsigned xg_t = sdfk_bx() / 8;
+    const unsigned tile = (((xg_t / SDFK_XGROUP) * 8 + sdfk_bx() % 8) * SDFK_XGROUP + xg_t % SDFK_XGROUP) * SDFK_RTILES + tt;
+    if (tile * SDFK_RNBRICK >= g.nbricks) break;
+    if (tt) __syncthreads();
+    unsigned rb, c;
+    sdfk_gbrick B[SDFK_RWBRICKS];
+    sdfk_rowsg_prepare(PRM, TAB, s, g, &meta, tile, rb, c, B);
+    const unsigned q0 = tile * SDFK_RNBRICK + wave * SDFK_RWBRICKS;
+#pragma unroll 1
+    for (int j = 0; j < SDFK_RWBRICKS; ++j) {
+        if (q0 + j >= g.nbricks) break;
+        const int b = wave * SDFK_RWBRICKS + j;
+        const unsigned k = c;
+        long long r0, rend;
+        sdfk_block_rows(g, rb, r0, rend);
+        if (++c == g.nchunk) { c = 0; ++rb; }
+        if (r0 >= rend) continue;
+        unsigned mw[2 * SDFK_NMASK];                             // the brick's skip bits as scalar words
+#pragma unroll
+        for (int w = 0; w < SDFK_NMASK; ++w) {
+            const unsigned long long m = meta.mask[w][b];
+            mw[2 * w] = __builtin_amdgcn_readfirstlane((unsigned)m);
+            mw[2 * w + 1] = __builtin_amdgcn_readfirstlane((unsigned)(m >> 32));
+        }
+        sdfk_gbrick cur = B[0];                                  // (one copy of the evaluation for both bricks)
+#pragma unroll
+        for (int t = 1; t < SDFK_RWBRICKS; ++t)
+            if (j == t) cur = B[t];
+        const bool uniform = sdfk_gbrick_uniform(cur);
+        const bool interior = sdfk_interior(g.L, k);
+#ifdef SDFK_ABLATE_EDGE
+        if (!interior) continue;
+#endif
+        const bool live_row = r0 + lr < rend;
+        const int dr = live_row ? lr : (int)(rend - 1 - r0);
+        long long f;                                              // flat index of this lane's first point
+        const int z = sdfk_win_z(r0 + dr, g.L, k, zq, &f);        // its index in the row (edge chunks: may lie outside)
+        const int last = (int)g.L - 1;
+        V3P P[SDFK_NP];
+        f2 res[SDFK_NP];
+#ifdef SDFK_FLAT
+        SDFK_EACH P[q].y = cur.w[q];
+#else
+        SDFK_EACH P[q].z = cur.w[q];
+#endif
+#ifdef SDFK_ABLATE_EVAL
+        if (true) {
+            SDFK_EACH res[q] = cur.w[q] + __builtin_bit_cast(float, mw[0] ^ mw[1] ^ mw[2] ^ mw[3]);
+        } else
+#endif
+        if (uniform) {
+#ifdef SDFK_FLAT
+            SDFK_EACH { P[q].x = sp<f2>(cur.x); P[q].z = sp<f2>(cur.y); }      // (x, 0)
+#else
+            SDFK_EACH { P[q].x = sp<f2>(cur.x); P[q].y = sp<f2>(cur.y); }
+#endif
+#ifndef SDFK_CHAIN
+            sdfk_rows_culled<true>(cur.x, cur.y, P, mw, PRM, TAB, res);
+#endif
+        } else {
+#ifdef SDFK_FLAT
+            SDFK_EACH { P[q].x = sp<f2>(cur.x); P[q].z = sp<f2>(cur.y); }
+#ifndef SDFK_CHAIN
+            sdfk_rows_culled<false>(0.0f, 0.0f, P, mw, PRM, TAB, res);
+#endif
+#endif
+        }
+#ifdef SDFK_CHAIN
+        {   // the children on the brick's list, in order; the first one starts the accumulator (parameters in SGPRs)
+            const unsigned cnt = __builtin_amdgcn_readfirstlane(meta.nalive[b]);
+            f2 acc[SDFK_NP];
+#pragma unroll 1
+            for (unsigned i = 0; i < cnt; ++i) {
+                const unsigned rec = __builtin_amdgcn_readfirstlane(sdfk_member_record((unsigned)meta.alist[b][i]));
+                f2 val[SDFK_NP];
+                SDFK_EACH val[q] = sdfk_leaf_rec<f2>(rec, P[q], PRM, TAB);
+                if (i == 0u) { SDFK_EACH acc[q] = val[q]; }
+                else { SDFK_EACH acc[q] = SDFK_CHAIN_CMB(acc[q], val[q], PRM); }
+            }
+            SDFK_EACH res[q] = sdfk_chain_tail<f2>(acc[q], P[q], PRM, TAB);
+        }
+#endif
+#ifdef SDFK_FLAGS                                                  // (the flag-writing build: the brick-tiled layout of sdfk_rows_kernel)
+        {
+            unsigned bits = 0u;
+            SDFK_EACH bits |= ((sdfk_sel_key(res[q].x) <= thr ? 1u : 0u) | (sdfk_sel_key(res[q].y) <= thr ? 2u : 0u)) << (2 * q);
+            if (!interior) {                                       // an edge window: only the points of this row
+                unsigned ok = 0u;
+                SDFK_EACH {
+                    if (z + 2 * q >= 0 && z + 2 * q <= last) ok |= 1u << (2 * q);
+                    if (z + 2 * q + 1 >= 0 && z + 2 * q + 1 <= last) ok |= 2u << (2 * q);
+                }
+                bits &= ok;
+            }
+            if (!live_row) bits = 0u;                              // rows past the end of the last block: empty slots
+            reinterpret_cast<unsigned char*>(flags)[(unsigned long long)(q0 + j) * 64ull + (unsigned)lane] = (unsigned char)bits;
+        }
+#else
+        if (live_row) {
+            float* po = out + f;
+            if (interior) {
+#pragma unroll
+                for (int q = 0; q < SDFK_NP; q += 2) {
+                    sdfk_f4u v = {res[q].x, res[q].y, res[q + 1].x, res[q + 1].y};
+                    __builtin_nontemporal_store(v, reinterpret_cast<sdfk_f4u*>(po + 2 * q));
+                }
+            } else {
+                SDFK_EACH {
+                    if (z + 2 * q >= 0 && z + 2 * q <= last) po[2 * q] = res[q].x;
+                    if (z + 2 * q + 1 >= 0 && z + 2 * q + 1 <= last) po[2 * q + 1] = res[q].y;
+                }
+            }
+        }
+#endif
+    }
+  }
+}
+#endif   // SDFK_GRID_BLOCKS
 #ifdef SDFK_WPE
 #define SDFK_ROWS_ATTR __attribute__((amdgpu_waves_per_eu(SDFK_WPE, SDFK_WPE)))
 #else
@@ -1707,7 +2108,11 @@
 extern "C" __global__ __launch_bounds__(64 * SDFK_RWAVES) void sdfk_spec_rg(
     const float* __restrict__ PRM, const float* __restrict__ TAB, SrcGrid s, sdfk_rowgeom g, float* __restrict__ out,
     unsigned* __restrict__ flags, unsigned thr SDFK_CELLS_KARG) {
+#ifdef SDFK_GRID_BLOCKS
+    sdfk_rowsg_kernel(PRM, TAB, s, g, out, flags, thr);
+#else
     sdfk_rows_kernel(PRM, TAB, s, g, out, flags, thr SDFK_CELLS_PASS);
+#endif
 }
 #ifdef SDFK_CELLS
 extern "C" __global__ __launch_bounds__(256) void sdfk_spec_cellsg(
@@ -2641,6 +3046,7 @@
         if (all || flat2 || flavour == SDFK_FL_ROWS_ARRAY || flavour == SDFK_FL_ROWS_GRID || flavour == SDFK_FL_ROWS_MASK) {
             g.s += kWaveHelpers;
             if (flat2) g.s += "\n#define SDFK_FLAT 1\n";
+            if (flavour == SDFK_FL_ROWS_GRID || flavour == SDFK_FL_ROWS2D_GRID) g.s += "\n#define SDFK_GRIDSRC 1\n";
             g.s += "\n#define SDFK_NP 4\n#define SDFK_EACH _Pragma(\"unroll\") for (int q = 0; q < SDFK_NP; ++q)\n"
                    "#define SDFK_NMASK 2\n"
                    "#define SDFK_SIMT 1\n#define SDFK_NSUB 1\n"
@@ -2696,6 +3102,7 @@
         g.n_root = 0;
         g.find_roots();
         if (flat) g.s += "\n#define SDFK_FLAT 1\n";
+        if (flavour == SDFK_FL_ROWS_GRID || flavour == SDFK_FL_ROWS2D_GRID) g.s += "\n#define SDFK_GRIDSRC 1\n";
         g.s += "\n#define SDFK_NP 4\n#define SDFK_EACH _Pragma(\"unroll\") for (int q = 0; q < SDFK_NP; ++q)\n";
         {
             char nm[64];
diff --git a/include/sdfk.h b/include/sdfk.h
--- a/include/sdfk.h
+++ b/include/sdfk.h
@@ -76,6 +76,7 @@
                                   const float* ax2, int64_t n2, int n_shards, const int* devices, int gather_device,
                                   float* d_full, int mode);
 void sdfk_set_default_mode(int mode);
+int sdfk_debug_grid_row(uint32_t row, uint32_t n1, uint32_t* ix, uint32_t* iy);
 int sdfk_debug_brick_masks(sdfk_program* prog, const float* d_co, int64_t n, int64_t row_stride, uint64_t* d_masks,
                            void* stream);
 int sdfk_debug_row_masks(sdfk_program* prog, const float* d_co, int64_t n, int64_t row_stride, int64_t row_len,
```
